# tauzn-clock/mpsfm

Measured on AMD Instinct MI355X. Metric: BA residual-evals/sec (LM iterations/sec alongside), 200 imgs / 150k pts prior-BA, higher is better.
Workload: dtype f64; 1 GPU; C3: 200 cameras, 150000 landmarks per rank, 749145 reprojection + 674306 log-depth blocks per rank, SoftL1/Cauchy, Ceres-default LM; parallelism=single GPU, residual_blocks_total=1423451

## Files before the change

### include/mpsfm_hip_debug.h

```cpp
#ifndef MPSFM_HIP_DEBUG_H
#define MPSFM_HIP_DEBUG_H

#include "mpsfm_hip.h"

#ifdef __cplusplus
extern "C" {
#endif

typedef struct mpsfm_plan_handle mpsfm_plan_handle;

void mpsfm_debug_set(int f);
int mpsfm_debug_set_chol_trace(long long* dev_buf);
int mpsfm_debug_panel_factor(const double* dx, int waves, double* out, int* ok);

mpsfm_plan_handle* mpsfm_debug_plan_create(const uint8_t* adj, int32_t n, int32_t depth, int32_t pinv_max_tiles, int32_t inv_rows);
void mpsfm_debug_plan_destroy(mpsfm_plan_handle* h);
int64_t mpsfm_debug_plan_get(const mpsfm_plan_handle* h, int32_t what, int32_t* out, int64_t cap);

int64_t mpsfm_debug_host_cache(int64_t bytes, int32_t count);
int64_t mpsfm_debug_run_parts(int32_t nparts, int32_t reps);
int mpsfm_debug_graph_union(const uint8_t* adj, int32_t world, int32_t n, uint8_t* out);

int mpsfm_debug_pt_handoff(mpsfm_ba_handle* h);
int mpsfm_debug_dense_solve_given(mpsfm_ba_handle* h, const double* S, const double* rhs, int32_t n, int32_t* failed);
int mpsfm_debug_read_trace(mpsfm_ba_handle* h, long long* out, int64_t count);
int64_t mpsfm_debug_table(mpsfm_ba_handle* h, int32_t which, void* out, int64_t cap);
int64_t mpsfm_debug_host_build(const mpsfm_ba_problem* P, int32_t which, void* out, int64_t cap);
int mpsfm_debug_local_clocks(mpsfm_ba_handle* h, int64_t out[12]);
int mpsfm_debug_local_skew(int32_t chunk, int32_t phase_mask, int64_t ticks);
int mpsfm_debug_resources(int32_t device, int64_t out[5]);

#ifdef __cplusplus
}
#endif
#endif
```

### mpsfm_amd/abi.py

```python

from __future__ import annotations

import ctypes as C
import os

MAX_TRACE = 64
INT_MAX_IRLS = 16

TERMINATION_NAMES = {
    0: "function_tolerance",
    1: "gradient_tolerance",
    2: "parameter_tolerance",
    3: "max_iterations",
    4: "min_radius",
    5: "invalid_steps",
    6: "no_variables",
}

ALLREDUCE_FN = C.CFUNCTYPE(C.c_int, C.c_void_p, C.POINTER(C.c_double), C.c_int64, C.c_int, C.c_void_p)


class CProblem(C.Structure):
    _c_name_ = "mpsfm_ba_problem"
    _fields_ = [
# ... 315 lines not shown

SIGNATURES = {
    "mpsfm_abi_version": (C.c_int, []),
    "mpsfm_last_error": (C.c_char_p, []),
    "mpsfm_device_count": (C.c_int, []),
    "mpsfm_ba_default_options": (None, [P]),
    "mpsfm_comm_unique_id": (C.c_int, [P]),
    "mpsfm_ba_solve": (C.c_int, [P, P, P, P]),
    "mpsfm_ba_create": (C.c_int, [P, P, P, _pp]),
    "mpsfm_ba_set_state": (C.c_int, [P, P]),
    "mpsfm_ba_reset_state": (C.c_int, [P]),
    "mpsfm_ba_solve_resident": (C.c_int, [P, P]),
    "mpsfm_ba_get_state": (C.c_int, [P, P]),
    "mpsfm_ba_destroy": (None, [P]),
    "mpsfm_ba_eval_cost": (C.c_int, [P, _f64p, _f64p]),
    "mpsfm_ba_sweep_once": (C.c_int, [P, F64, _f32p]),
    "mpsfm_ba_sweep_parts": (C.c_int, [P, P, P]),
    "mpsfm_ba_get_reduced_system": (C.c_int, [P, P, P, I32]),
    "mpsfm_ba_reduced_dim": (C.c_int, [P]),
    "mpsfm_ba_get_dense_solution": (C.c_int, [P, P, I32]),
    "mpsfm_ba_dense_solve_once": (C.c_int, [P, _f32p]),
    "mpsfm_ba_dense_plan": (C.c_int, [P, P]),
    "mpsfm_point_covs": (C.c_int, [P, P, I32, P]),
    "mpsfm_triangulate_tracks": (C.c_int, [P, I32, P]),
    "mpsfm_filter_tracks": (C.c_int, [P, P, I32, P, P, P]),
    "mpsfm_tri_default_options": (None, [P]),
    "mpsfm_triangulator_create": (C.c_int, [P, I32, _pp]),
    "mpsfm_triangulator_destroy": (None, [P]),
    "mpsfm_triangulator_set_state": (C.c_int, [P, P]),
    "mpsfm_triangulator_triangulate_image": (C.c_int, [P, P, I32, _i64p]),
    "mpsfm_triangulator_complete_image": (C.c_int, [P, P, I32, _i64p]),
    "mpsfm_triangulator_complete_tracks": (C.c_int, [P, P, P, I64, _i64p]),
    "mpsfm_triangulator_merge_tracks": (C.c_int, [P, P, P, I64, _i64p]),
    "mpsfm_triangulator_retriangulate": (C.c_int, [P, P, P, I32, _i64p]),
    "mpsfm_triangulator_num_ops": (I64, [P]),
    "mpsfm_triangulator_num_points": (I64, [P]),
    "mpsfm_triangulator_get_ops": (C.c_int, [P, P, P, P, P]),
    "mpsfm_triangulator_num_op_elements": (I64, [P]),
    "mpsfm_triangulator_get_op_elements": (C.c_int, [P, P]),
    "mpsfm_triangulator_stats": (C.c_int, [P, _i64p, _i64p, _i64p]),
    "mpsfm_tri_estimate_batch": (C.c_int, [P, I32, P, P, P]),
    "mpsfm_depth_blocks": (C.c_int, [P, I32, P, P, P, P, P, P]),
    "mpsfm_integrate_depth": (C.c_int, [P, I32, P, P]),
    "mpsfm_integrate_depth_batch": (C.c_int, [I32, P, I32, P, P]),
    "mpsfm_integration_variances": (C.c_int, [P, I32, I32, I32, P, P, F64, I32, P, P, P]),
    "mpsfm_depth_consistency": (C.c_int, [I32, P, I32, P, P, F64, F64, I32, P, P, P]),
    "mpsfm_abs_pose_estimate": (C.c_int, [I64, P, P, P, P, I32, P, P]),
    "mpsfm_rel_pose_estimate": (C.c_int, [I64, P, P, P, P, P, I32, P, P]),
    "mpsfm_two_view_default_options": (None, [P]),
    "mpsfm_two_view_geometry": (C.c_int, [I64, P, P, P, P, P, P, P, I32, P, P]),
    "mpsfm_two_view_geometry_batch": (C.c_int, [I64, P, P, P, P, P, P, P, P, I32, I32, P, P, P]),
    "mpsfm_registration_pairs": (C.c_int, [I32, P, I64, P, P, P, P, I32, P, I32, I32, P, P, P]),
    "mpsfm_init_pair_candidates": (C.c_int, [P, I32, P]),
    "mpsfm_radius_nms": (C.c_int, [I64, P, P, P, F64, I32, P, P, P]),
    "mpsfm_thin_dense_matches": (C.c_int, [I64, P, P, I64, P, P, P, F64, I32, I32, P, P, P]),
    "mpsfm_assign_keypoints": (C.c_int, [I64, P, I64, P, F64, I32, P, P]),
    "mpsfm_match_default_options": (None, [P]),
    "mpsfm_match_descriptors": (C.c_int, [I64, I64, I32, P, P, P, I32, P, P, P]),
    "mpsfm_match_descriptors_batch": (C.c_int, [I32, P, I32, P, I64, P, P, P, P, I32, I32, I32, P, P, P, P]),
    "mpsfm_match_map_descriptors": (C.c_int, [P, P, I32, I32, P, P, I32, I32, I32, I64, P, I64, P, P, I32, P, P, P]),
    "mpsfm_recip_default_options": (None, [P]),
    "mpsfm_recip_seed_count": (I64, [I32, I32, I32]),
    "mpsfm_reciprocal_nns": (C.c_int, [P, I32, I32, P, I32, I32, I32, P, I32, I64, P, P, P, P]),
    "mpsfm_dense_correspondences": (C.c_int, [P, P, P, P, P, P, P, P, I32, I32, I32, I32, I32, P, I32, I64, P, P, P, P, P]),
    "mpsfm_warp_default_options": (None, [P]),
    "mpsfm_simple_nms": (C.c_int, [I32, I32, P, I32, I32, P, I32, P, P]),
    "mpsfm_kpids_to_matches0": (C.c_int, [I64, P, P, P, I64, I64, I32, P, I32, P, P, P, P]),
    "mpsfm_warp_matches": (C.c_int, [I32, I32, P, P, I32, I32, I32, I32, I32, P, I64, P, I64, P, I32, P, P, P, P, P, P, P, P]),
    "mpsfm_depth_priors": (C.c_int, [I32, P, P, I32, P, P]),
    "mpsfm_normal_priors": (C.c_int, [I32, P, P, I32, P, P]),
}

DEBUG_SIGNATURES = {
    "mpsfm_debug_set": (None, [C.c_int]),
    "mpsfm_debug_set_chol_trace": (C.c_int, [P]),
    "mpsfm_debug_panel_factor": (C.c_int, [P, C.c_int, P, C.POINTER(C.c_int)]),
    "mpsfm_debug_plan_create": (P, [P, I32, I32, I32, I32]),
    "mpsfm_debug_plan_destroy": (None, [P]),
    "mpsfm_debug_plan_get": (I64, [P, I32, P, I64]),
    "mpsfm_debug_host_cache": (I64, [I64, I32]),
    "mpsfm_debug_run_parts": (I64, [I32, I32]),
    "mpsfm_debug_graph_union": (C.c_int, [P, I32, I32, P]),
    "mpsfm_debug_pt_handoff": (C.c_int, [P]),
    "mpsfm_debug_dense_solve_given": (C.c_int, [P, P, P, I32, C.POINTER(I32)]),
    "mpsfm_debug_read_trace": (C.c_int, [P, P, I64]),
    "mpsfm_debug_table": (I64, [P, I32, P, I64]),
    "mpsfm_debug_host_build": (I64, [P, I32, P, I64]),
    "mpsfm_debug_local_clocks": (C.c_int, [P, P]),
    "mpsfm_debug_local_skew": (C.c_int, [I32, I32, I64]),
    "mpsfm_debug_resources": (C.c_int, [I32, P]),
}


LIB_PATH = os.path.join(os.path.dirname(os.path.abspath(__file__)), "libmpsfm_hip.so")

_lib = None


class MpsfmHipError(RuntimeError):
    def __init__(self, code: int, msg: str):
        super().__init__(f"libmpsfm_hip error {code}: {msg}")
        self.code = code


def lib():
    global _lib
    if _lib is None:
        if not os.path.exists(LIB_PATH):
            raise MpsfmHipError(-2, f"{LIB_PATH} is missing: run `python -m mpsfm_amd.build` (hipcc, gfx950)")
        try:
            import torch
        except ImportError:
            pass
        L = C.CDLL(LIB_PATH)
        for table in (SIGNATURES, DEBUG_SIGNATURES):
            for name, (restype, argtypes) in table.items():
                fn = getattr(L, name)
                fn.restype, fn.argtypes = restype, argtypes
        _lib = L
    return _lib
```

### mpsfm_amd/capi.py

```python

from __future__ import annotations

import ctypes as C

import numpy as np

from .abi import (
    ALLREDUCE_FN, LIB_PATH, SIGNATURES, CAbsPoseOptions, CAbsPoseResult, CDcImage, CDcSummary, CDepthGather, CDepthPriorConf,
    CDepthPriorOutput, CDepthPriorProblem, CInitCandidates, CInitPair, CIntProblem, CIntSummary, CMatchBatchReport, CMatchInfo, CMatchOptions, CNmsInfo,
    CNormalPriorConf, CNormalPriorOutput, CNormalPriorProblem, COptions, CPriorSummary, CProblem, CRansacOptions, CRecipInfo,
    CRecipOptions, CRegImage, CRelPoseOptions, CRelPoseResult, CState, CSummary, CTracks, CTriCandidates, CTwoViewBatchReport, CTwoViewLeg, CTwoViewOptions,
    CTwoViewResult, CWarpInfo, CWarpOptions, MpsfmHipError, lib,
)
from .problem import BAProblem, Tracks

EXPORTS = list(SIGNATURES)
_MATCH_DESC_ARGS = SIGNATURES["mpsfm_match_descriptors"][1]
_MATCH_MAP_ARGS = SIGNATURES["mpsfm_match_map_descriptors"][1]
_SIMPLE_NMS_ARGS = SIGNATURES["mpsfm_simple_nms"][1]
_KPIDS_ARGS = SIGNATURES["mpsfm_kpids_to_matches0"][1]
_WARP_ARGS = SIGNATURES["mpsfm_warp_matches"][1]


def _check(rc: int):
# ... 37 lines not shown
_open_handles: "weakref.WeakSet" = None


def _track(handle):
    global _open_handles
    import atexit
    import weakref

    if _open_handles is None:
        _open_handles = weakref.WeakSet()

        def _close_all():
            for h in list(_open_handles):
                try:
                    h.close()
                except Exception:
                    pass

        atexit.register(_close_all)
    _open_handles.add(handle)


class BAHandle:

    def __init__(self, prob: BAProblem, options: COptions | None = None):
        self._h = C.c_void_p(None)
        self.prob = prob
        self.options = options if options is not None else default_options()
        cp, cs = prob.c_problem(), prob.c_state()
        _check(lib().mpsfm_ba_create(C.byref(cp), C.byref(cs), C.byref(self.options), C.byref(self._h)))
        _track(self)

    def close(self):
        if self._h:
            lib().mpsfm_ba_destroy(self._h)
            self._h = C.c_void_p(None)

    def __del__(self):
        try:
            self.close()
        except Exception:
            pass

    def __enter__(self):
        return self

    def __exit__(self, *a):
        self.close()

    def set_state(self, prob: BAProblem | None = None):
        cs = (prob or self.prob).c_state()
        _check(lib().mpsfm_ba_set_state(self._h, C.byref(cs)))

    def reset_state(self):
        _check(lib().mpsfm_ba_reset_state(self._h))

    def solve(self) -> dict:
        sm = CSummary()
        _check(lib().mpsfm_ba_solve_resident(self._h, C.byref(sm)))
        return sm.to_dict()

    def get_state(self, prob: BAProblem | None = None):
        cs = (prob or self.prob).c_state()
        _check(lib().mpsfm_ba_get_state(self._h, C.byref(cs)))

    def eval_cost(self) -> tuple[float, float]:
        a, b = C.c_double(0), C.c_double(0)
        _check(lib().mpsfm_ba_eval_cost(self._h, C.byref(a), C.byref(b)))
        return a.value, b.value

    @property
    def reduced_dim(self) -> int:
        return int(lib().mpsfm_ba_reduced_dim(self._h))

    def dense_plan(self) -> dict:
        v = (C.c_int64 * 10)()
        _check(lib().mpsfm_ba_dense_plan(self._h, v))
        keys = ["slots", "tile_columns", "levels", "nd_depth", "inverse_accumulators", "work_items", "tile_products", "inverse_roles",
                "s_blocks", "backsub_launches"]
        return dict(zip(keys, (int(x) for x in v)))

    def pt_handoff(self) -> bool:
        return bool(lib().mpsfm_debug_pt_handoff(self._h))

    def sweep_once(self, radius: float = 1e4) -> float:
        ms = C.c_float(0)
        _check(lib().mpsfm_ba_sweep_once(self._h, radius, C.byref(ms)))
        return ms.value

    def sweep_parts(self) -> dict:
        ms, info = (C.c_float * 3)(), (C.c_int64 * 4)()
        _check(lib().mpsfm_ba_sweep_parts(self._h, ms, info))
        return dict(dense_ms=ms[0], reduce_ms=ms[1], general_ms=ms[2], dense_chunks=int(info[0]), general_chunks=int(info[1]),
                    long_tracks=int(info[2]), reduce_parts=int(info[3]))

    def dense_solve_once(self) -> float:
        ms = C.c_float(0)
        _check(lib().mpsfm_ba_dense_solve_once(self._h, C.byref(ms)))
        return ms.value

    def dense_solve_given(self, S: np.ndarray, rhs: np.ndarray) -> bool:
        n = self.reduced_dim
        S, rhs = np.ascontiguousarray(S, np.float64), np.ascontiguousarray(rhs, np.float64)
        assert S.shape == (n, n) and rhs.shape == (n,)
        failed = C.c_int32(0)
        _check(lib().mpsfm_debug_dense_solve_given(self._h, S.ctypes.data, rhs.ctypes.data, n, C.byref(failed)))
        return bool(failed.value)

    def reduced_system(self):
        n = self.reduced_dim
        S, rhs = np.zeros((n, n)), np.zeros(n)
        _check(lib().mpsfm_ba_get_reduced_system(self._h, S.ctypes.data, rhs.ctypes.data, n))
        return S, rhs

    def dense_solution(self):
        n = self.reduced_dim
        y = np.zeros(n)
        _check(lib().mpsfm_ba_get_dense_solution(self._h, y.ctypes.data, n))
        return y


def ba_solve(prob: BAProblem, options: COptions | None = None) -> dict:
    o = options if options is not None else default_options()
    cp, cs, sm = prob.c_problem(), prob.c_state(), CSummary()
    _check(lib().mpsfm_ba_solve(C.byref(cp), C.byref(cs), C.byref(o), C.byref(sm)))
    return sm.to_dict()


def point_covs(prob: BAProblem, device: int = 0) -> np.ndarray:
    covs = np.zeros((prob.n_pts, 3, 3))
    cp, cs = prob.c_problem(), prob.c_state()
    _check(lib().mpsfm_point_covs(C.byref(cp), C.byref(cs), device, covs.ctypes.data))
    return covs


def debug_panel_factor(dx: np.ndarray, waves: int = 4):
    dx = np.ascontiguousarray(dx, np.float64)
    assert dx.shape == (64, 32), dx.shape
    out, ok = np.zeros((64, 32)), C.c_int(0)
    _check(lib().mpsfm_debug_panel_factor(dx.ctypes.data, int(waves), out.ctypes.data, C.byref(ok)))
    return out, bool(ok.value)


def debug_resources(device: int = 0) -> tuple:
    out = np.zeros(5, np.int64)
    _check(lib().mpsfm_debug_resources(int(device), out.ctypes.data))
    return tuple(int(v) for v in out)


def triangulate_tracks(tr: Tracks, device: int = 0) -> np.ndarray:
    xyz = np.zeros((tr.n_tracks, 3))
    ct = tr.c_tracks()
    _check(lib().mpsfm_triangulate_tracks(C.byref(ct), device, xyz.ctypes.data))
    return xyz


def filter_tracks(tr: Tracks, xyz: np.ndarray, device: int = 0):
    xyz = np.ascontiguousarray(xyz, np.float64)
    ang, err, front = np.zeros(tr.n_tracks), np.zeros(tr.n_el), np.zeros(tr.n_el, np.uint8)
    ct = tr.c_tracks()
    _check(lib().mpsfm_filter_tracks(C.byref(ct), xyz.ctypes.data, device, ang.ctypes.data, err.ctypes.data, front.ctypes.data))
    return ang, err, front.astype(bool)


def depth_blocks(depth_maps, valid_maps, sx, sy, cam_quat, cam_t, obs_img, obs_xy, obs_var, obs_pt, pts, scale_filter_factor=1.5,
                 multiplier=2.0, device=0):
# ... 938 lines not shown
```

### mpsfm_amd/csrc/ba_build.hip

```cpp
#include <algorithm>
#include <chrono>
#include <cstdio>
#include <cstring>
#include <mutex>
#include <string>
#include <vector>

#include "ba_handle.h"

namespace mpsfm {

void free_handle(mpsfm_ba_handle* h) {
  if (!h) return;
  (void)hipSetDevice(h->device);
  comm_destroy(h->comm);
  delete h;
}

int check_problem(const mpsfm_ba_problem* P) {
  if (!P) return fail(MPSFM_EINVAL, "problem is NULL");
  if (P->n_cams < 0 || P->n_pts < 0 || P->n_intr < 0 || P->n_obs < 0 || P->n_dobs < 0) return fail(MPSFM_EINVAL, "negative size");
  if (P->n_cams > 0 && (!P->cam_intr_idx || !P->pose_const || !P->cam_intr)) return fail(MPSFM_EINVAL, "camera arrays are NULL");
  if (P->n_pts > 0 && !P->pt_const) return fail(MPSFM_EINVAL, "pt_const is NULL");
  if (P->n_obs > 0 && (!P->obs_cam || !P->obs_pt || !P->obs_xy)) return fail(MPSFM_EINVAL, "observation arrays are NULL");
  if (P->n_dobs > 0 && (!P->dobs_cam || !P->dobs_pt || !P->dobs_depth || !P->dobs_magnitude || !P->dobs_param))
    return fail(MPSFM_EINVAL, "depth observation arrays are NULL");
  if (P->gauge_axis_cam < -1 || P->gauge_axis_cam >= P->n_cams) return fail(MPSFM_EINVAL, "gauge_axis_cam out of range");
  for (int i = 0; i < P->n_cams; ++i)
    if (P->cam_intr_idx[i] < 0 || P->cam_intr_idx[i] >= P->n_intr) return fail(MPSFM_EINVAL, "cam_intr_idx out of range");
  auto out_of_range = [](const int32_t* v, int64_t n, int32_t bound) {
    uint32_t bad = 0;
    const uint32_t b = (uint32_t)bound;
    for (int64_t i = 0; i < n; ++i) bad |= (uint32_t)((uint32_t)v[i] >= b);
    return bad != 0;
  };
  if (out_of_range(P->obs_cam, P->n_obs, P->n_cams) || out_of_range(P->obs_pt, P->n_obs, P->n_pts))
    return fail(MPSFM_EINVAL, "observation index out of range");
  if (out_of_range(P->dobs_cam, P->n_dobs, P->n_cams) || out_of_range(P->dobs_pt, P->n_dobs, P->n_pts))
    return fail(MPSFM_EINVAL, "depth observation index out of range");
  for (int t : {P->reproj_loss_type, P->depth_loss_type})
    if (t < MPSFM_LOSS_TRIVIAL || t > MPSFM_LOSS_CAUCHY) return fail(MPSFM_EINVAL, "unknown loss type");
  return 0;
}

void level_plan_flags(const CholPlan& PL, LevelPlanDev& D) { D.valid = PL.nt >= 1 && PL.nlevels >= 1; D.use_pinv = PL.use_pinv; }

static int upload_pattern(mpsfm_ba_handle* h, bool use_graph) {
  const CholPlan& PL = h->plan;
  DeviceBlocks& own = h->own;
  h->sky.ns = h->ncv;
  if (int rc = use_graph ? own.upload(&h->sky.index, h->spat.sky_index) : own.upload(&h->sky.first, h->spat.sky_first, &h->sky.start, h->spat.sky_start))
    return rc;
  std::vector<uint8_t> live((size_t)(PL.nt + 1) * (size_t)(PL.nt + 2) / 2, 0);
  for (int32_t id : PL.asm_tiles) live[(size_t)id] = 1;
  LevelPlanDev& D = h->lp;
  if (int rc = own.upload(&D.d_items, PL.items, &D.d_heads, PL.heads, &D.d_srcs, PL.srcs, &D.d_rows, PL.rows, &D.d_struct_start, PL.struct_start,
                          &D.d_struct_rows, PL.struct_rows, &D.d_back_cols, PL.back_cols, &D.d_asm_tiles, PL.asm_tiles,
                          &D.d_col_slot, PL.slot_of_col, &D.d_tile_live, live))
    return rc;
  if (PL.slot_of_col.empty()) D.d_col_slot = nullptr;
  level_plan_flags(PL, D);
  D.n_asm = (int32_t)PL.asm_tiles.size(); D.nlevels = PL.nlevels;
  D.h_launch_start = PL.launch_start.data(); D.h_back_start = PL.back_start.data();
  return 0;
}


static void graph_from_stage1(const std::vector<uint64_t>& gbits, int words, const std::vector<int32_t>& prov, int nprov, const CameraLayout& cams,
                              CamGraph& graph) {
  graph.init(cams.ncv_real);
  std::vector<int32_t> nat_of_prov((size_t)std::max(nprov, 1), -1);
  for (size_t i = 0; i < cams.slot.size(); ++i) if (prov[i] >= 0) nat_of_prov[(size_t)prov[i]] = cams.slot[i];
  for (int a = 0; a < nprov; ++a) {
    const int na = nat_of_prov[(size_t)a];
    for (int w = 0; w < words; ++w) {
      uint64_t m = gbits[(size_t)a * words + w];
      while (m) {
        const int b = w * 64 + __builtin_ctzll(m);
        m &= m - 1;
        const int nb = nat_of_prov[(size_t)b];
        if (na >= 0 && nb >= 0) graph.set(na, nb);
      }
    }
  }
}

static int pair_tables_of_device_build(hipStream_t stream, const mpsfm_ba_problem* P, const RecTablesDev& rt, HostTables& T, const Lap& lap) {
  std::vector<ChunkHdr>& chunks = T.chunks;
  size_t g0 = 0;
  while (g0 < chunks.size() && chunks[g0].dense) ++g0;
  T.blk_ent_start.assign(g0, 0);
  if (g0 == chunks.size()) return 0;
  const int64_t r0 = chunks[g0].rec0, k0 = chunks[g0].pt0, nrg = T.nrec - r0, nkg = T.np_chunked - k0;
  std::vector<uint32_t> rm((size_t)std::max<int64_t>(nrg, 1));
  std::vector<uint16_t> kvs((size_t)std::max<int64_t>(nkg, 1));
  std::vector<int32_t> prs((size_t)std::max<int64_t>(nkg, 1));
  MPSFM_TRY(hipMemcpyAsync(rm.data(), rt.rec_meta + r0, 4 * (size_t)nrg, hipMemcpyDeviceToHost, stream));
  MPSFM_TRY(hipMemcpyAsync(kvs.data(), rt.pt_kv + k0, 2 * (size_t)nkg, hipMemcpyDeviceToHost, stream));
  MPSFM_TRY(hipMemcpyAsync(prs.data(), rt.pt_rec_start + k0, 4 * (size_t)nkg, hipMemcpyDeviceToHost, stream));
  MPSFM_TRY(hipStreamSynchronize(stream));
  PairScratch ps;
  for (size_t c = g0; c < chunks.size(); ++c) {
    if (chunks[c].dense) return fail(MPSFM_EUNSUPPORTED, "internal: dense chunks must precede the general ones");
    append_pair_tables(chunks[c], rm.data() - r0, kvs.data() - k0, prs.data() - k0, T.order.data(), P->pt_const, T.blk_desc, T.ents, T.blk_ent_start, ps);
  }
  if (T.ents.size() > (size_t)INT32_MAX) return fail(MPSFM_EUNSUPPORTED, "too many Schur pairs for 32-bit entry offsets");
  lap("pair tables of the general chunks (host)");
  return 0;
}

static void print_chunk_stats(const std::vector<ChunkHdr>& chunks) {
  double sr = 0, sp = 0, sc = 0, sb = 0, se = 0, sd = 0; int mb = 0, mc = 0;
  for (const ChunkHdr& H : chunks) { sr += H.nrec; sp += H.npt; sc += H.ncam; sb += H.nblk; se += H.nent; sd += H.dense; mb = std::max(mb, H.nblk); mc = std::max(mc, H.ncam); }
  const double n = (double)chunks.size();
  std::fprintf(stderr, "[mpsfm_ba] build: %zu chunks; per chunk: %.1f records, %.1f landmarks, %.1f cameras (max %d), %.1f work items (max %d), %.1f pairs; %.0f %% of the chunks take the dense product\n",
               chunks.size(), sr / n, sp / n, sc / n, mc, sb / n, mb, se / n, 100.0 * sd / n);
  int hist[kDenseCams + 2] = {0};
  for (const ChunkHdr& H : chunks) ++hist[std::min<int>(H.ncam, kDenseCams + 1)];
  std::fprintf(stderr, "[mpsfm_ba] build: chunks by number of variable cameras:");
  for (int c = 0; c <= kDenseCams + 1; ++c) std::fprintf(stderr, " %s%d: %d", c > kDenseCams ? ">" : "", c > kDenseCams ? kDenseCams : c, hist[c]);
  std::fprintf(stderr, "\n");
}

static int upload_tables(mpsfm_ba_handle* h, const mpsfm_ba_problem* P, const CameraLayout& cams, DevBuildOut& DB, SlabTables& R, DevBuilder* devb,
                         bool slab_tables_on_device) {
  HostTables& T = DB.t;
  const int nc = P->n_cams;
  int rc = 0;
  DeviceBlocks& own = h->own;
  std::vector<double> intr(P->cam_intr, P->cam_intr + (size_t)P->n_intr * 4);
  std::vector<int32_t> intr_idx(P->cam_intr_idx, P->cam_intr_idx + nc);
  if ((rc = own.upload(&h->d_intr, intr, &h->d_intr_idx, intr_idx, &h->d_cmask, cams.cmask, &h->d_cam_slot, h->cam_slot_h,
                       &h->d_cam_of_slot, cam_of_slot_table(cams), &h->d_chunks, T.chunks, &h->d_chunk_cams, T.chunk_cams)))
    return rc;
  if (h->np > 0 && h->np == (int64_t)h->np_user) {
    if ((rc = own.upload(&h->d_perm, h->perm))) return rc;
    if ((rc = own.alloc(&h->d_user_pts, (size_t)h->np * 3))) return rc;
  }
  if (h->built_on_device) {
    h->rt = DB.rt;
    own.adopt(std::move(DB.own));
    own.drop(DB.d_chunks); own.drop(DB.d_chunk_cams);
  } else {
    RecTablesDev& rt = h->rt;
    if ((rc = own.upload(&rt.rec_cam, T.rec_cam, &rt.rec_pt, T.rec_pt, &rt.rec_meta, T.rec_meta, &rt.rec_xy, T.rec_xy, &rt.rec_d, T.rec_d, &rt.rec_m, T.rec_m,
                         &rt.rec_a, T.rec_a, &rt.pt_rec_start, T.pt_rec_start, &rt.pt_kv, T.pt_kv, &rt.fx_cam, T.fx_cam, &rt.fx_pt, T.fx_pt,
                         &rt.fx_meta, T.fx_meta, &rt.fx_xy, T.fx_xy, &rt.fx_d, T.fx_d, &rt.fx_m, T.fx_m, &rt.fx_a, T.fx_a)))
      return rc;
  }
  if ((rc = own.upload(&h->d_lhdr, T.lhdr))) return rc;
  if ((rc = own.alloc(&h->d_wl, (size_t)std::max<int64_t>(T.wl_rows, 1) * 18))) return rc;
  h->n_blk_desc = (int64_t)T.blk_desc.size(); h->n_blk_ent_start = (int64_t)T.blk_ent_start.size(); h->n_ents = (int64_t)T.ents.size();
  if ((rc = own.upload(&h->d_blk_desc, T.blk_desc, &h->d_blk_ent_start, T.blk_ent_start, &h->d_ents, T.ents))) return rc;
  int32_t* d_diag_block = nullptr;
  if (!slab_tables_on_device) {
    if ((rc = own.upload(&h->d_red_dests, R.dests, &h->d_red_srcs, R.srcs))) return rc;
  } else if ((rc = own.upload(&d_diag_block, R.diag_block))) return rc;
  if ((rc = own.alloc(&h->d_slab, (size_t)std::max<int64_t>(R.slab_units, 1) * 18))) return rc;

  if ((rc = staged_drain())) return rc;
  if (slab_tables_on_device) {
    if ((rc = devb->slab_tables(h->d_chunks, h->n_dense, h->d_chunk_cams, h->sky, h->spat.nblk, h->ncv, d_diag_block, own, &h->d_red_dests, &h->n_red_dests,
                                &h->d_red_srcs, &h->n_red_srcs)))
      return rc;
    MPSFM_TRY(hipStreamSynchronize(h->stream));
    own.drop(d_diag_block);
  }
  return 0;
}

static int alloc_work_buffers(mpsfm_ba_handle* h, const BuildOptions& opt) {
  int rc = 0;
  DeviceBlocks& own = h->own;
  const size_t ncs = (size_t)std::max(h->nc, 1), nps = (size_t)std::max<int64_t>(h->np, 1);
  for (double** p : {&h->d_q, &h->d_q2, &h->d_q0}) if ((rc = own.alloc(p, ncs * 4))) return rc;
  for (double** p : {&h->d_t, &h->d_t2, &h->d_t0}) if ((rc = own.alloc(p, ncs * 3))) return rc;
  for (double** p : {&h->d_pts, &h->d_pts2, &h->d_pts0, &h->d_ps, &h->d_diagV}) if ((rc = own.alloc(p, nps * 3))) return rc;
  if (h->nlong == 0 && h->n_dense > 0 && h->n_dense == h->nchunks) if ((rc = own.alloc(&h->d_pt_fac, nps * 9))) return rc;
  if ((rc = own.alloc(&h->d_cs, ncs * 6))) return rc;
  if ((rc = own.alloc(&h->d_camtab, ncs * kCamRec))) return rc;
  if ((rc = own.alloc(&h->d_camtab2, ncs * kCamRec))) return rc;
  h->sblk_count = h->spat.nblk * 36;
  h->red_count = h->sblk_count + 3 * (int64_t)h->n_user + SC_COUNT;
  if ((rc = own.alloc(&h->d_red, (size_t)h->red_count))) return rc;
  h->d_Sblk = h->d_red; h->d_gc = h->d_red + h->sblk_count; h->d_wv = h->d_gc + h->n_user; h->d_diagU = h->d_wv + h->n_user;
  h->d_redsc = h->d_diagU + h->n_user;
  if ((rc = own.alloc(&h->d_part, (size_t)std::max(h->nchunks + h->nlong, 1) * 4 * 2))) return rc;
  if ((rc = own.alloc(&h->d_part2, (size_t)std::max(h->nchunks + h->nlong, 1) * 8))) return rc;
  if ((rc = own.alloc(&h->d_scal, (size_t)U_COUNT))) return rc;
  if ((rc = own.alloc(&h->d_costpart, (size_t)1024 * 4))) return rc;
  static_assert(sizeof(double) * U_COUNT * 2 <= kPinnedBytes, "pinned scalar block too small");
  MPSFM_TRY(own.pinned((void**)&h->h_scal));
  static_assert(sizeof(LmCtl) * 2 <= kPinnedBytes, "pinned block too small for two control-block copies");
  MPSFM_TRY(own.pinned((void**)&h->h_ctl));
  if ((rc = own.alloc(&h->d_ctl, 1))) return rc;
  for (auto& e : h->ev2) MPSFM_TRY(own.event(&e, true));
  const size_t ntiles = (size_t)(h->nt + 1) * (h->nt + 2) / 2;
  if ((rc = own.alloc(&h->d_A, ntiles * 1024))) return rc;
  if ((rc = own.alloc(&h->d_dwork, dense_work_doubles(h->nt)))) return rc;
  if ((rc = own.alloc(&h->d_yc, (size_t)std::max(h->n_user, 1)))) return rc;
  if ((rc = own.alloc(&h->d_fail, 1))) return rc;
  MPSFM_TRY(hipMemsetAsync(h->d_fail, 0, sizeof(int), h->stream));
  for (auto& e : h->ev) MPSFM_TRY(own.event(&e, true));
  opt.apply_dense(h->nt, h->plan, h->ov);
  if (h->nt > 64 || h->ov.nb > 0) {
    MPSFM_TRY(own.stream(&h->ov.s2));
    for (auto& e : h->ov.evF) MPSFM_TRY(own.event(&e, false));
    for (auto& e : h->ov.evB) MPSFM_TRY(own.event(&e, false));
  }
  h->local_ok = false;
  if (opt.local_lm && !sharded(h) && h->nlong == 0 && h->nchunks > 0 && h->n_dense == h->nchunks && h->ncv >= 1 && h->ncv <= kLocalCams &&
      h->n_user == 6 * h->ncv && h->nchunks <= local_lm_max_chunks(h->device)) {
    h->local_log_cap = std::max(h->opt.max_num_iterations, 0) + 2;
    if ((rc = own.alloc(&h->d_local_acc, (size_t)2 * kLocalAccDoubles))) return rc;
    if ((rc = own.alloc(&h->d_local_sync, (size_t)16))) return rc;
    if ((rc = own.alloc(&h->d_local_log, (size_t)h->local_log_cap))) return rc;
    h->local_ok = true;
  }
  MPSFM_TRY(hipMemsetAsync(h->d_ps, 0, nps * 3 * sizeof(double), h->stream));
  MPSFM_TRY(hipMemsetAsync(h->d_yc, 0, (size_t)std::max(h->n_user, 1) * sizeof(double), h->stream));
  MPSFM_TRY(hipStreamSynchronize(h->stream));
  return 0;
}

int build_tables(const mpsfm_ba_problem* P, BuildOptions& opt, const SumExchange& exchange, bool sharded, int verbose, const Lap& lap, DeviceStages* devs,
                 TableBuild& out) {
  const int nc = P->n_cams;
  CameraLayout& cams = out.cams;
  HostTables& T = out.tables.t;

  bool dev = false;
  std::vector<uint64_t> dev_gbits;
  std::vector<int32_t> prov((size_t)std::max(nc, 1), -1);
  int nprov = 0;
  for (int i = 0; i < nc; ++i) if (!P->pose_const[i]) prov[(size_t)i] = nprov++;
  const int dev_words = (nprov + 63) / 64;
  std::vector<double> cnt(nc + 1, 0.0);
  if (devs && !sharded && nprov <= kIndexMaxSlots && nc <= 8192 && P->n_obs + P->n_dobs > 0 && opt.dev_build && opt.chol_graph) {
    devs->builder.reset(new DevBuilder());
    int64_t max_blocks = 0;
    if (int rc = devs->builder->stage1(P, devs->stream, prov, nprov, cnt, dev_gbits, dev_words, &max_blocks)) return rc;
    dev = max_blocks <= kObsMax;
    lap("device stage 1 (upload, group, graph)");
  } else {
    count_camera_blocks(P, cnt);
    if (exchange) if (int rc = exchange(cnt.data(), nc)) return rc;
  }
  assign_camera_slots(P, cnt, opt, cams);
  opt.set_chunk_caps(sharded, cams.ncv, P->n_obs);

  LandmarkGroups groups;
  if (!dev) if (int rc = group_blocks_by_landmark(P, true, groups)) return rc;
  lap("group blocks by landmark (threads)");

  CamGraph graph;
  if (cams.use_graph) {
    if (dev) graph_from_stage1(dev_gbits, dev_words, prov, nprov, cams, graph);
    else camera_graph_from_groups(P, groups, cams, graph);
    if (exchange) if (int rc = union_graph_over_ranks(graph, exchange)) return rc;
    lap("camera graph");
    plan_camera_order(graph, opt, out.plan, cams);
    lap("camera order + factorisation plan");
  } else keep_caller_order(cams);

  if (dev) {
    const int rc2 = devs->builder->stage2(cams.slot, opt.sweep_dense, opt.rec_cap, opt.pts_by_cams, out.tables);
    if (rc2 < 0) return rc2;
    if (rc2 == MPSFM_DEVBUILD_FALLBACK) {
      dev = false;
      if (int rc = group_blocks_by_landmark(P, false, groups)) return rc;
      lap("device build not applicable: host phases");
    } else {
      if (T.nrec > (int64_t)INT32_MAX) return fail(MPSFM_EUNSUPPORTED, "more than 2^31 records on one device");
      lap("device stage 2 (order, chunks, records)");
      if (int rc = pair_tables_of_device_build(devs->stream, P, out.tables.rt, T, lap)) return rc;
    }
  }
  if (!dev) if (int rc = build_record_tables(P, cams, opt, groups, T, lap)) return rc;
  out.built_on_device = dev;
  {
    double tot[3] = {(double)(P->n_obs + P->n_dobs), (double)T.nblk_reduced, T.nvarpts};
    if (exchange) if (int rc = exchange(tot, 3)) return rc;
    out.nblocks_global = tot[0]; out.nblocks_reduced_global = tot[1]; out.nvarpts_global = tot[2];
  }
  lap("chunks + pair tables");
  if (verbose >= 2 && !T.chunks.empty()) print_chunk_stats(T.chunks);

  if (cams.use_graph) s_pattern_index(cams, out.plan, graph, out.spat);
  else if (int rc = s_pattern_skyline(cams, T, opt, exchange, verbose >= 2, out.spat, out.plan)) return rc;
  if (verbose >= 2) {
    const CholPlan& PL = out.plan;
    std::fprintf(stderr, "[mpsfm_ba] build: camera order: %s (depth %d), %d slots for %d cameras, %d tile columns in %d levels, %lld tile products, %lld inverse roles, %d blocks of S\n",
                 PL.nd_depth < 0 ? "caller's" : "nested dissection", PL.nd_depth, PL.nslots, PL.ncv, PL.nt, PL.nlevels, (long long)PL.products, (long long)PL.roles, (int)out.spat.nblk);
  }

  SlabTables& slabs = out.slabs;
  if (int rc = assign_slabs(T.chunks, slabs)) return rc;
  out.slab_tables_on_device = dev && slabs.n_dense > 0 && (opt.slab_tables_host == 0 || (opt.slab_tables_host < 0 && slabs.n_dense >= 512));
  if (int rc = slab_reduction_tables(T, cams, out.plan, out.spat, !out.slab_tables_on_device, slabs)) return rc;
  lap("slab reduction tables");
  return 0;
}

static int build(mpsfm_ba_handle* h, const mpsfm_ba_problem* P) {
  const Lap lap = stopwatch(h->opt.verbose >= 2, "[mpsfm_ba] build: %-28s %8.2f ms\n");
  h->nc = P->n_cams; h->np_user = P->n_pts;
  h->loss.reproj_type = P->reproj_loss_type; h->loss.reproj_a = P->reproj_loss_scale;
  h->loss.reproj_mag = P->reproj_loss_magnitude; h->loss.depth_type = P->depth_loss_type;
  BuildOptions opt = BuildOptions::from_environment();
  const SumExchange exchange = sharded(h) ? SumExchange([h](double* buf, int64_t count) { return allreduce_host(h, buf, count); }) : SumExchange();
  DeviceStages devs{h->stream, nullptr};
  TableBuild B;
  if (int rc = build_tables(P, opt, exchange, sharded(h), h->opt.verbose, lap, &devs, B)) return rc;

  h->plan = std::move(B.plan); h->spat = std::move(B.spat);
  const CameraLayout& cams = B.cams;
  HostTables& T = B.tables.t;
  h->n_user = 6 * cams.ncv_real;
  h->cam_slot_h = cams.slot; h->nat_slot = cams.nat_slot;
  h->ncv = cams.ncv; h->n = cams.n; h->nt = cams.nt;
  h->built_on_device = B.built_on_device;
  h->np = T.np; h->np_chunked = T.np_chunked; h->nfixed = T.nfixed; h->nrec = T.nrec;
  h->nchunks = (int)T.chunks.size(); h->nlong = (int)T.lhdr.size();
  h->nblocks_total = P->n_obs + P->n_dobs; h->nblocks_reduced = T.nblk_reduced;
  h->nblocks_global = B.nblocks_global; h->nblocks_reduced_global = B.nblocks_reduced_global; h->nvarpts_global = B.nvarpts_global;
  h->n_dense = B.slabs.n_dense; h->n_red_dests = (int)B.slabs.dests.size();
  h->n_red_srcs = (int64_t)B.slabs.srcs.size(); h->n_chunk_cams = (int64_t)T.chunk_cams.size();
  h->perm.swap(T.order);

  if (int rc = upload_pattern(h, cams.use_graph)) return rc;
  if (int rc = upload_tables(h, P, cams, B.tables, B.slabs, devs.builder.get(), B.slab_tables_on_device)) return rc;
  lap("upload tables");
  if (int rc = alloc_work_buffers(h, opt)) return rc;
  lap("allocate work buffers");
  return 0;
}

int upload_state(mpsfm_ba_handle* h, const mpsfm_ba_state* st, bool as_initial) {
  if (!st || (h->nc > 0 && (!st->cam_quat_xyzw || !st->cam_t)) || (h->np > 0 && !st->pts)) return fail(MPSFM_EINVAL, "state is NULL");
  const Lap lap = stopwatch(h->opt.verbose >= 2, "[mpsfm_ba] state: %-28s %8.2f ms\n");
  MPSFM_TRY(hipStreamSynchronize(h->stream));
  lap("stream idle");
  if (h->nc > 0) {
    if (int rc = staged_h2d(h->d_q, st->cam_quat_xyzw, sizeof(double) * 4 * h->nc)) return rc;
    if (int rc = staged_h2d(h->d_t, st->cam_t, sizeof(double) * 3 * h->nc)) return rc;
  }
  lap("pose copies");
  if (h->d_perm) {
    if (int rc = staged_h2d(h->d_user_pts, st->pts, sizeof(double) * 3 * h->np)) return rc;
    launch_permute_pts(h->np, h->d_perm, h->d_user_pts, h->d_pts, false, h->stream);
    lap("landmark copy + permute (device)");
  } else {
    std::vector<double> sorted((size_t)h->np * 3);
    parallel_ranges(h->np, 16384, [&](int64_t k0, int64_t k1) {
      for (int64_t k = k0; k < k1; ++k) {
        const double* s = st->pts + 3 * (size_t)h->perm[(size_t)k];
        sorted[3 * (size_t)k] = s[0]; sorted[3 * (size_t)k + 1] = s[1]; sorted[3 * (size_t)k + 2] = s[2];
      }
    });
    lap("permute landmarks");
    if (h->np > 0) if (int rc = staged_h2d(h->d_pts, sorted.data(), sizeof(double) * 3 * h->np)) return rc;
  }
  lap("landmark copy");
  if (as_initial) {
    MPSFM_TRY(hipMemcpyAsync(h->d_q0, h->d_q, sizeof(double) * 4 * h->nc, hipMemcpyDeviceToDevice, h->stream));
    MPSFM_TRY(hipMemcpyAsync(h->d_t0, h->d_t, sizeof(double) * 3 * h->nc, hipMemcpyDeviceToDevice, h->stream));
    if (h->np > 0) MPSFM_TRY(hipMemcpyAsync(h->d_pts0, h->d_pts, sizeof(double) * 3 * h->np, hipMemcpyDeviceToDevice, h->stream));
    MPSFM_TRY(hipStreamSynchronize(h->stream));
    lap("keep initial state");
  }
  h->scales_ready = false;
  return 0;
}

int create_impl(const mpsfm_ba_problem* P, const mpsfm_ba_state* st, const mpsfm_ba_options* o, mpsfm_ba_handle** out) {
  if (!out) return fail(MPSFM_EINVAL, "out is NULL");
  *out = nullptr;
  const auto t_begin = std::chrono::steady_clock::now();
  auto since = [&](const char* what) {
    if (o && o->verbose >= 2)
      std::fprintf(stderr, "[mpsfm_ba] create: %-27s %8.2f ms (cumulative)\n", what,
                   1e3 * std::chrono::duration<double>(std::chrono::steady_clock::now() - t_begin).count());
  };
  if (int rc = check_problem(P)) return rc;
  if (!o) return fail(MPSFM_EINVAL, "options is NULL");
  since("check_problem");
  int ndev = 0;
  if (hipGetDeviceCount(&ndev) != hipSuccess || ndev <= 0) return fail(MPSFM_ENODEVICE, "no HIP device visible: libmpsfm_hip has no CPU fallback");
  if (o->device < 0 || o->device >= ndev) return fail(MPSFM_EINVAL, "device ordinal out of range");
  if (o->device >= kMaxDevices) return fail(MPSFM_EUNSUPPORTED, "device ordinals beyond 15 are not supported (per-device pools)");
  {
    static std::mutex mu;
    static std::vector<std::string> arch;
    std::lock_guard<std::mutex> lk(mu);
    if ((int)arch.size() < ndev) arch.resize((size_t)ndev);
    if (arch[(size_t)o->device].empty()) {
      hipDeviceProp_t prop;
      MPSFM_TRY(hipGetDeviceProperties(&prop, o->device));
      arch[(size_t)o->device] = prop.gcnArchName;
    }
    if (std::strncmp(arch[(size_t)o->device].c_str(), "gfx950", 6) != 0)
      return fail(MPSFM_ENODEVICE, std::string("device is ") + arch[(size_t)o->device] + ", this library is built for gfx950 only");
  }
  since("device check");
  MPSFM_TRY(hipSetDevice(o->device));
  mpsfm_ba_handle* h = new mpsfm_ba_handle();
  h->device = o->device; h->opt = *o;
  if (o->stream) { h->stream = (hipStream_t)o->stream; h->own.idle_first(h->stream); }
  else if (h->own.stream(&h->stream) != hipSuccess) { delete h; return fail(MPSFM_EHIP, "hipStreamCreate failed"); }
  if (o->use_rccl && o->world_size >= 1) {
    if (int rc = comm_init_rank(h)) { free_handle(h); return rc; }
    since("ncclCommInitRank");
  }
  int rc = build(h, P);
  since("build");
  if (rc == 0 && st) rc = upload_state(h, st, true);
  since("upload_state");
// ... 7 lines not shown
```

### mpsfm_amd/csrc/ba_debug.hip

```cpp
#include <algorithm>
#include <atomic>
#include <cstring>
#include <vector>

#include "../../include/mpsfm_hip_debug.h"
#include "ba_handle.h"

using namespace mpsfm;

static void dense_plan_numbers(int ncv, int nt, const CholPlan& P, const DenseOverlap& ov, const LevelPlanDev& lp, double* work, int64_t sblk, int64_t v[10]) {
  const bool level = dense_level(&ov, &lp);
  const bool pinv = level && dense_pinv(work, nt, &ov, &lp) != nullptr;
  const int64_t w[10] = {ncv, nt, level ? P.nlevels : nt, P.nd_depth, pinv ? 1 : 0, (int64_t)P.items.size(), P.products, P.roles, sblk,
                         pinv ? 1 : (level ? P.nlevels : (nt + 3) / 4 + 1)};
  for (int i = 0; i < 10; ++i) v[i] = w[i];
}

extern "C" int64_t mpsfm_debug_host_cache(int64_t bytes, int32_t count) {
  std::vector<mpsfm::HostBuf<uint8_t>> first((size_t)count), second((size_t)count);
  std::vector<const void*> seen;
  for (auto& b : first) { b.alloc((size_t)bytes); b[0] = 1; b[(size_t)bytes - 1] = 2; seen.push_back(b.data()); }
  first.clear();
  int64_t reused = 0;
  for (auto& b : second) {
    b.alloc((size_t)bytes);
    b[0] = 3;
    reused += std::find(seen.begin(), seen.end(), (const void*)b.data()) != seen.end() ? 1 : 0;
  }
  return reused;
}

extern "C" int64_t mpsfm_debug_run_parts(int32_t nparts, int32_t reps) {
  int64_t bad = 0;
  for (int r = 0; r < reps; ++r) {
    std::vector<std::atomic<int>> hits((size_t)std::max(nparts, 1));
    for (auto& x : hits) x.store(0);
    mpsfm::run_parts(nparts, [&](int t, int np) {
      if (np != std::max(nparts, 1) || t < 0 || t >= np) return;
      volatile double acc = 0.0;
      for (int k = 0; k < 2000; ++k) acc = acc + (double)k * 1e-9;
      hits[(size_t)t].fetch_add(1);
    });
    for (auto& x : hits) bad += x.load() == 1 ? 0 : 1;
  }
  return bad;
}

extern "C" int mpsfm_debug_graph_union(const uint8_t* adj, int32_t world, int32_t n, uint8_t* out) {
  std::vector<double> sum;
  for (int r = 0; r < world; ++r) {
    mpsfm::CamGraph g;
    g.init(n);
    for (int a = 0; a < n; ++a)
      for (int b = 0; b < n; ++b)
        if (adj[((size_t)r * n + a) * n + b]) g.set(a, b);
    std::vector<double> packed;
    mpsfm::pack_graph(g, world, packed);
    if (sum.empty()) sum.assign(packed.size(), 0.0);
    for (size_t i = 0; i < packed.size(); ++i) sum[i] += packed[i];
  }
  mpsfm::CamGraph u;
  u.init(n);
  mpsfm::unpack_graph(sum, world, u);
  for (int a = 0; a < n; ++a)
    for (int b = 0; b < n; ++b) out[(size_t)a * n + b] = u.get(a, b) ? 1 : 0;
  return mpsfm::graph_digits(world);
}

extern "C" {

int mpsfm_ba_dense_plan(mpsfm_ba_handle* h, int64_t info[10]) {
  if (!h || !info) return fail(MPSFM_EINVAL, "handle or info is NULL");
  dense_plan_numbers(h->ncv, h->nt, h->plan, h->ov, h->lp, h->d_dwork, h->spat.nblk, info);
  return 0;
}

int mpsfm_debug_pt_handoff(mpsfm_ba_handle* h) { return h && h->d_pt_fac != nullptr ? 1 : 0; }

int mpsfm_ba_sweep_once(mpsfm_ba_handle* h, double radius, float* elapsed_ms) {
  if (!h) return fail(MPSFM_EINVAL, "handle is NULL");
  MPSFM_TRY(hipSetDevice(h->device));
  if (!h->scales_ready) if (int rc = prepare_scales(h)) return rc;
  MPSFM_TRY(hipMemsetAsync(h->d_red, 0, sizeof(double) * (size_t)h->red_count, h->stream));
  SweepArgs a = sweep_args(h, radius);
  MPSFM_TRY(hipEventRecord(h->ev[0], h->stream));
  launch_track_sweep_dense(a, h->n_dense, h->stream);
  MPSFM_TRY(hipEventRecord(h->ev[1], h->stream));
  launch_reduce_slabs(h->d_red_dests, h->n_red_dests, h->d_red_srcs, h->d_slab, h->d_Sblk, h->d_gc, h->d_wv, h->d_diagU, nullptr, h->stream);
  MPSFM_TRY(hipEventRecord(h->ev[2], h->stream));
  a.chunk0 = h->n_dense;
  launch_track_sweep(a, h->nchunks - h->n_dense, false, h->stream);
  MPSFM_TRY(hipEventRecord(h->ev[3], h->stream));
  if (h->nchunks + h->nlong > 0) launch_reduce_cols(h->d_part, h->nchunks + h->nlong, 4, 3, 1u << 2, h->d_redsc, h->stream);
  MPSFM_TRY(hipStreamSynchronize(h->stream));
  MPSFM_TRY(hipGetLastError());
  h->last_radius = radius;
  float ms = 0.f;
  MPSFM_TRY(hipEventElapsedTime(&ms, h->ev[0], h->ev[3]));
  if (elapsed_ms) *elapsed_ms = ms;
  return 0;
}

int mpsfm_debug_read_trace(mpsfm_ba_handle* h, long long* out, int64_t count) {
  if (!h || !out || count < 0 || count > 3 * std::max<int64_t>(h->np, 1)) return fail(MPSFM_EINVAL, "bad trace request");
  MPSFM_TRY(hipSetDevice(h->device));
  MPSFM_TRY(hipMemcpyAsync(out, h->d_diagV, sizeof(long long) * (size_t)count, hipMemcpyDeviceToHost, h->stream));
  MPSFM_TRY(hipStreamSynchronize(h->stream));
  return 0;
}

int64_t mpsfm_debug_table(mpsfm_ba_handle* h, int32_t which, void* out, int64_t cap) {
  if (!h) return fail(MPSFM_EINVAL, "handle is NULL");
  const void* src = nullptr;
  int64_t bytes = 0;
  bool host = false;
  const int64_t nr = h->nrec, np1 = h->np + 1, nf = h->nfixed;
  switch (which) {
    case 0: src = h->d_chunks; bytes = (int64_t)sizeof(ChunkHdr) * h->nchunks; break;
    case 1: src = h->d_chunk_cams; bytes = 4 * h->n_chunk_cams; break;
    case 2: src = h->rt.rec_cam; bytes = 4 * nr; break;
    case 3: src = h->rt.rec_pt; bytes = 4 * nr; break;
    case 4: src = h->rt.rec_meta; bytes = 4 * nr; break;
    case 5: src = h->rt.rec_xy; bytes = 16 * nr; break;
    case 6: src = h->rt.rec_d; bytes = 8 * nr; break;
    case 7: src = h->rt.rec_m; bytes = 8 * nr; break;
    case 8: src = h->rt.rec_a; bytes = 8 * nr; break;
    case 9: src = h->rt.pt_rec_start; bytes = 4 * np1; break;
    case 10: src = h->rt.pt_kv; bytes = 2 * np1; break;
    case 11: src = h->rt.fx_cam; bytes = 4 * nf; break;
    case 12: src = h->rt.fx_pt; bytes = 4 * nf; break;
    case 13: src = h->rt.fx_meta; bytes = 4 * nf; break;
    case 14: src = h->rt.fx_xy; bytes = 16 * nf; break;
    case 15: src = h->rt.fx_d; bytes = 8 * nf; break;
    case 16: src = h->rt.fx_m; bytes = 8 * nf; break;
    case 17: src = h->rt.fx_a; bytes = 8 * nf; break;
    case 18: src = h->perm.data(); bytes = 4 * (int64_t)h->perm.size(); host = true; break;
    case 19: src = h->d_red_dests; bytes = (int64_t)sizeof(RedDest) * h->n_red_dests; break;
    case 20: src = h->d_red_srcs; bytes = 4 * h->n_red_srcs; break;
    case 21: src = h->cam_slot_h.data(); bytes = 4 * (int64_t)h->cam_slot_h.size(); host = true; break;
    case 23: src = h->d_blk_desc; bytes = 4 * h->n_blk_desc; break;
    case 24: src = h->d_blk_ent_start; bytes = 4 * h->n_blk_ent_start; break;
    case 25: src = h->d_ents; bytes = 4 * h->n_ents; break;
    case 26: src = h->d_part; bytes = 32 * (int64_t)h->nchunks; break;
    case 22: { static uint8_t flag; flag = h->built_on_device ? 1 : 0; src = &flag; bytes = 1; host = true; break; }
    case 27: src = h->d_lhdr; bytes = (int64_t)sizeof(LongHdr) * h->nlong; break;
    case 28: src = h->spat.sky_index.data(); bytes = 4 * (int64_t)h->spat.sky_index.size(); host = true; break;
    case 29: src = h->spat.sky_first.data(); bytes = 4 * (int64_t)h->spat.sky_first.size(); host = true; break;
    case 30: src = h->spat.sky_start.data(); bytes = 8 * (int64_t)h->spat.sky_start.size(); host = true; break;
    case 31: src = h->d_cmask; bytes = 48 * (int64_t)h->nc; break;
    case 32: src = h->d_cam_of_slot; bytes = 4 * (int64_t)std::max(h->ncv, 1); break;
    case 33: { static thread_local int64_t info[10]; if (int rc = mpsfm_ba_dense_plan(h, info)) return rc; src = info; bytes = 80; host = true; break; }
    case 34: src = h->last_launches; bytes = (int64_t)sizeof(h->last_launches); host = true; break;
    default: return fail(MPSFM_EINVAL, "unknown table");
  }
  if (!out || cap < bytes) return bytes;
  if (bytes == 0) return 0;
  if (host) { std::memcpy(out, src, (size_t)bytes); return bytes; }
  if (hipSetDevice(h->device) != hipSuccess) return fail(MPSFM_EHIP, "hipSetDevice failed");
  if (hipMemcpyAsync(out, src, (size_t)bytes, hipMemcpyDeviceToHost, h->stream) != hipSuccess) return fail(MPSFM_EHIP, "copy failed");
  if (hipStreamSynchronize(h->stream) != hipSuccess) return fail(MPSFM_EHIP, "sync failed");
// ... 184 lines not shown
```

### mpsfm_amd/csrc/ba_handle.h

```cpp
#pragma once
#include <cstdint>
#include <memory>
#include <vector>

#include "ba_launch.h"
#include "build_host.h"
#include "common.h"
#include "dev_resources.h"
#include "devbuild.h"

struct mpsfm_ba_handle {
  int device = 0;
  mpsfm::DeviceBlocks own;
  hipStream_t stream = nullptr;
  void* comm = nullptr;
  mpsfm::DenseOverlap ov;
  mpsfm::SPattern spat;
  mpsfm::BlockSky sky{nullptr, nullptr, nullptr, 0};
  mpsfm::CholPlan plan;
  mpsfm::LevelPlanDev lp;
  std::vector<int32_t> nat_slot;
  int n_user = 0;
  mpsfm_ba_options opt{};
  mpsfm::LossParams loss{};
  int nc = 0, np_user = 0;
  int64_t np = 0, np_chunked = 0;
  int64_t nrec = 0, nfixed = 0, nblocks_total = 0, nblocks_reduced = 0;
  double nblocks_global = 0, nblocks_reduced_global = 0, nvarpts_global = 0;
  int ncv = 0, n = 0, nt = 0, nchunks = 0, nlong = 0;
  int n_dense = 0;
  double* d_slab = nullptr;
  mpsfm::RedDest* d_red_dests = nullptr;
  int32_t* d_red_srcs = nullptr;
  int n_red_dests = 0;
  int64_t n_red_srcs = 0, n_chunk_cams = 0, n_blk_desc = 0, n_blk_ent_start = 0, n_ents = 0;
  bool built_on_device = false;
  mpsfm::LongHdr* d_lhdr = nullptr;
  double* d_wl = nullptr;
  int64_t red_count = 0, sblk_count = 0;
  std::vector<int32_t> perm;
  int32_t* d_cam_of_slot = nullptr;
  int32_t* d_perm = nullptr;
  double* d_user_pts = nullptr;
  std::vector<int32_t> cam_slot_h;
  double *d_q = nullptr, *d_t = nullptr, *d_q2 = nullptr, *d_t2 = nullptr, *d_q0 = nullptr, *d_t0 = nullptr;
  double *d_pts = nullptr, *d_pts2 = nullptr, *d_pts0 = nullptr;
  double *d_intr = nullptr, *d_cmask = nullptr, *d_cs = nullptr, *d_camtab = nullptr, *d_camtab2 = nullptr;
  int32_t *d_intr_idx = nullptr, *d_cam_slot = nullptr;
  double *d_ps = nullptr, *d_diagV = nullptr;
  double* d_pt_fac = nullptr;
  mpsfm::ChunkHdr* d_chunks = nullptr;
  int32_t *d_chunk_cams = nullptr, *d_blk_ent_start = nullptr;
  uint32_t *d_blk_desc = nullptr, *d_ents = nullptr;
  mpsfm::RecTablesDev rt;
  double* d_red = nullptr;
  double *d_Sblk = nullptr, *d_gc = nullptr, *d_wv = nullptr, *d_diagU = nullptr, *d_redsc = nullptr;
  double *d_part = nullptr, *d_part2 = nullptr, *d_scal = nullptr, *d_costpart = nullptr;
  double* h_scal = nullptr;
  mpsfm::LmCtl* d_ctl = nullptr;
  mpsfm::LmCtl* h_ctl = nullptr;
  hipEvent_t ev2[4] = {nullptr, nullptr, nullptr, nullptr};
  double *d_A = nullptr, *d_yc = nullptr, *d_dwork = nullptr;
  int* d_fail = nullptr;
  hipEvent_t ev[4] = {nullptr, nullptr, nullptr, nullptr};
  double last_radius = 1e4;
  bool scales_ready = false;
  int64_t last_launches[mpsfm::kLfCount] = {};
  double split_front_s = 0.0;
  bool local_ok = false;
  double* d_local_acc = nullptr;
  int64_t* d_local_sync = nullptr;
  mpsfm::LmHead* d_local_log = nullptr;
  int local_log_cap = 0;
};

namespace mpsfm {

inline bool sharded(const mpsfm_ba_handle* h) { return h->opt.allreduce != nullptr || h->comm != nullptr; }

struct TableBuild {
  CameraLayout cams;
  CholPlan plan;
  SPattern spat;
  DevBuildOut tables;
  SlabTables slabs;
  double nblocks_global = 0, nblocks_reduced_global = 0, nvarpts_global = 0;
  bool built_on_device = false;
  bool slab_tables_on_device = false;
};
struct DeviceStages {
  hipStream_t stream = nullptr;
  std::unique_ptr<DevBuilder> builder;
};

int check_problem(const mpsfm_ba_problem* P);
int build_tables(const mpsfm_ba_problem* P, BuildOptions& opt, const SumExchange& exchange, bool sharded, int verbose, const Lap& lap, DeviceStages* dev,
                 TableBuild& out);
void level_plan_flags(const CholPlan& PL, LevelPlanDev& D);

int create_impl(const mpsfm_ba_problem* P, const mpsfm_ba_state* st, const mpsfm_ba_options* o, mpsfm_ba_handle** out);
int upload_state(mpsfm_ba_handle* h, const mpsfm_ba_state* st, bool as_initial);
void free_handle(mpsfm_ba_handle* h);

int comm_init_rank(mpsfm_ba_handle* h);
void comm_destroy(void* comm);
int allreduce_host(mpsfm_ba_handle* h, double* buf, int64_t count);
int allreduce_dev(mpsfm_ba_handle* h, double* buf, int64_t count);

SweepArgs sweep_args(mpsfm_ba_handle* h, double radius, const LmCtl* ctl = nullptr);
int prepare_scales(mpsfm_ba_handle* h);
int run_track_sweep(mpsfm_ba_handle* h, double radius, const LmCtl* ctl = nullptr, bool in_loop = false, bool adopt = false, bool handoff = false);
void run_assemble(mpsfm_ba_handle* h, double radius, const LmCtl* ctl = nullptr);
int run_dense(mpsfm_ba_handle* h, double radius, const LmCtl* ctl = nullptr);
bool chol_entry_list();

struct LocalSkew { int32_t chunk = 0, mask = 0; int64_t ticks = 0; };
extern LocalSkew g_local_skew;

}
```

### mpsfm_amd/csrc/ba_launch.h

```cpp
#pragma once
#include "common.h"
#include "local_lm.h"

namespace mpsfm {
enum LaunchFamily {
  kLfTrackSweep,
  kLfReduceSlabs,
  kLfAssemble,
  kLfCholLevel,
  kLfDenseRest,
  kLfUpdateSweep,
  kLfDecide,
  kLfScales,
  kLfOther,
  kLfCount
};
extern thread_local int64_t g_launches[kLfCount];
inline void count_launch(LaunchFamily f, int n = 1) { g_launches[f] += n; }

void launch_track_sweep(const SweepArgs&, int nchunks, bool diag_only, hipStream_t);
void launch_update_sweep(const SweepArgs&, int nchunks, hipStream_t, const CamUpdArgs* cu = nullptr);
void launch_track_sweep_dense(const SweepArgs&, int nchunks, hipStream_t);
void launch_reduce_slabs(const RedDest* dests, int ndest, const int32_t* srcs, const double* slab, double* Sblk, double* gc, double* wv, double* diagU,
                         const LmCtl* ctl, hipStream_t);
void launch_cost_records(const CostArgs&, int nblocks, hipStream_t);
void launch_reduce_cols(const double* part, int64_t rows, int stride, int ncols, uint32_t max_mask, double* out, hipStream_t,
                        double* out2 = nullptr, int gmax_slot = -1);
void launch_build_camtab(int nc, const double* q, const double* t, const double* intr, const int32_t* intr_idx,
                         const double* cs, double* camtab, hipStream_t);
void launch_cam_scales(int nc, const int32_t* cam_slot, const double* cmask, const double* diagU, int jacobi, double* cs, hipStream_t);
void launch_pt_scales(int64_t np, const uint16_t* pt_kv, const double* diagV, int jacobi, double* ps, hipStream_t);
void launch_cam_update(int nc, const int32_t* cam_slot, const double* q, const double* t, const double* cs, const double* yc,
                       const double* gc, double* q2, double* t2, double* scal, hipStream_t, const double* intr = nullptr,
                       const int32_t* intr_idx = nullptr, double* camtab2 = nullptr, int* chol_fail = nullptr, const LmCtl* ctl = nullptr);
void launch_lm_decide(LmCtl* ctl, double* scal, const LmOpts& o, LmCtl* host_copy, hipStream_t, const double* redsc = nullptr);
void launch_zero(double* p, int64_t n, const LmCtl* ctl, hipStream_t);
void launch_lm_reduce_decide(const double* part, const double* part2, int64_t rows, LmCtl* ctl, double* scal, const LmOpts& o, LmCtl* host_copy, hipStream_t);
void launch_lm_prologue(const LmCtl* ctl, double* red, int64_t nred, int nc, int64_t np, double* q, double* t, double* camtab, double* pts, const double* q2,
                        const double* t2, const double* camtab2, const double* pts2, hipStream_t);
void launch_lm_accept(const LmCtl* ctl, int nc, int64_t np, double* q, double* t, double* camtab, double* pts, const double* q2, const double* t2,
                      const double* camtab2, const double* pts2, hipStream_t);
void launch_pts_sqnorm(int64_t np, const uint16_t* pt_kv, const double* pts, double* part, int nblocks, hipStream_t);
void launch_gmax_to_slot(double* redsc, int rank, hipStream_t);
void launch_lm_pack(const double* scal, double* sums, hipStream_t);
void launch_lm_init(LmCtl* ctl, const double* scal, const double* sums, hipStream_t);
void launch_permute_pts(int64_t np, const int32_t* perm, const double* src, double* dst, bool scatter, hipStream_t);
void launch_gmax_from_slots(const double* redsc, double* scal, hipStream_t);

extern int g_dbg_flags;
void launch_assemble(const AssembleArgs&, hipStream_t);
void launch_dense_solve(double* A, double* work, int nt, int n, double* y, int* fail, hipStream_t, DenseOverlap* ov, const LevelPlanDev* lp,
                        const LmCtl* ctl = nullptr);
bool dense_level(const DenseOverlap* ov, const LevelPlanDev* lp);
int dense_plain_max_tiles();
int dense_inv_rows();
size_t dense_work_doubles(int nt);
double* dense_pinv(double* work, int nt, const DenseOverlap* ov, const LevelPlanDev* lp);

int local_lm_max_chunks(int device);
int launch_local_lm(const LocalArgs& a, hipStream_t s);

}
```

### mpsfm_amd/csrc/ba_solver.hip

```cpp
#include <algorithm>
#include <chrono>
#include <cstdio>
#include <cstdlib>
#include <cstring>
#include <vector>

#include "ba_handle.h"

namespace mpsfm {

LocalSkew g_local_skew;

SweepArgs sweep_args(mpsfm_ba_handle* h, double radius, const LmCtl* ctl) {
  SweepArgs a{};
  a.ctl = ctl;
  a.chunks = h->d_chunks; a.chunk_cams = h->d_chunk_cams; a.rec_cam = h->rt.rec_cam; a.rec_meta = h->rt.rec_meta;
  a.rec_xy = h->rt.rec_xy; a.rec_d = h->rt.rec_d; a.rec_m = h->rt.rec_m; a.rec_a = h->rt.rec_a;
  a.pt_rec_start = h->rt.pt_rec_start; a.pt_kv = h->rt.pt_kv; a.blk_desc = h->d_blk_desc; a.blk_ent_start = h->d_blk_ent_start; a.ents = h->d_ents;
  a.camtab = h->d_camtab; a.pts = h->d_pts; a.ps = h->d_ps; a.loss = h->loss;
  a.radius = radius; a.min_diag = h->opt.min_lm_diagonal; a.max_diag = h->opt.max_lm_diagonal; a.ncv = h->ncv; a.dbg = (g_dbg_flags >> 8) & 0xff;
  a.lhdr = h->d_lhdr; a.nlong = h->nlong; a.nchunks = h->nchunks; a.cam_slot = h->d_cam_slot; a.wl = h->d_wl;
  a.sky = h->sky;
  a.Sblk = h->d_Sblk; a.gc = h->d_gc; a.wv = h->d_wv; a.diagU = h->d_diagU; a.part = h->d_part; a.diagV = h->d_diagV;
  a.yc = h->d_yc; a.camtab2 = h->d_camtab2; a.pts2 = h->d_pts2; a.part2 = h->d_part2;
  a.slab = h->d_slab; a.chunk0 = 0;
  return a;
}

static void launch_record_cost(mpsfm_ba_handle* h, bool fixed, double* out) {
  const RecTablesDev& r = h->rt;
  const int64_t nrec = fixed ? h->nfixed : h->nrec;
  const int nb = (int)std::min<int64_t>(1024, (nrec + kThreads - 1) / kThreads);
  const CostArgs c = fixed ? CostArgs{nrec, r.fx_cam, r.fx_pt, r.fx_meta, r.fx_xy, r.fx_d, r.fx_m, r.fx_a, h->d_camtab, h->d_pts, h->loss, h->d_costpart}
                           : CostArgs{nrec, r.rec_cam, r.rec_pt, r.rec_meta, r.rec_xy, r.rec_d, r.rec_m, r.rec_a, h->d_camtab, h->d_pts, h->loss, h->d_costpart};
  launch_cost_records(c, nb, h->stream);
  launch_reduce_cols(h->d_costpart, nb, 4, 3, 0u, out, h->stream);
}
static void launch_fixed_cost(mpsfm_ba_handle* h, double* out) {
  if (h->nfixed > 0) launch_record_cost(h, true, out);
}
static int cost_of_records(mpsfm_ba_handle* h, bool fixed, double* out3) {
  out3[0] = out3[1] = out3[2] = 0.0;
  if ((fixed ? h->nfixed : h->nrec) <= 0) return 0;
  launch_record_cost(h, fixed, h->d_scal);
  MPSFM_TRY(hipMemcpyAsync(h->h_scal, h->d_scal, sizeof(double) * 3, hipMemcpyDeviceToHost, h->stream));
  MPSFM_TRY(hipStreamSynchronize(h->stream));
  out3[0] = h->h_scal[0]; out3[1] = h->h_scal[1]; out3[2] = h->h_scal[2];
  return 0;
}

int prepare_scales(mpsfm_ba_handle* h) {
  hipStream_t s = h->stream;
  launch_cam_scales(h->nc, h->d_cam_slot, h->d_cmask, h->d_diagU, 0, h->d_cs, s);
  launch_pt_scales(h->np, h->rt.pt_kv, h->d_diagV, 0, h->d_ps, s);
  launch_build_camtab(h->nc, h->d_q, h->d_t, h->d_intr, h->d_intr_idx, h->d_cs, h->d_camtab, s);
  if (h->opt.jacobi_scaling) {
    MPSFM_TRY(hipMemsetAsync(h->d_diagU, 0, sizeof(double) * (size_t)std::max(h->n_user, 1), s));
    MPSFM_TRY(hipMemsetAsync(h->d_diagV, 0, sizeof(double) * 3 * (size_t)std::max<int64_t>(h->np, 1), s));
    SweepArgs a = sweep_args(h, 1.0);
    launch_track_sweep(a, h->nchunks, true, s);
    if (int rc = allreduce_dev(h, h->d_diagU, h->n_user)) return rc;
    launch_cam_scales(h->nc, h->d_cam_slot, h->d_cmask, h->d_diagU, 1, h->d_cs, s);
    launch_pt_scales(h->np, h->rt.pt_kv, h->d_diagV, 1, h->d_ps, s);
    launch_build_camtab(h->nc, h->d_q, h->d_t, h->d_intr, h->d_intr_idx, h->d_cs, h->d_camtab, s);
  }
  MPSFM_TRY(hipGetLastError());
  h->scales_ready = true;
  return 0;
}

static void launch_sweeps(mpsfm_ba_handle* h, SweepArgs a, hipStream_t s) {
  launch_track_sweep_dense(a, h->n_dense, s);
  launch_reduce_slabs(h->d_red_dests, h->n_red_dests, h->d_red_srcs, h->d_slab, h->d_Sblk, h->d_gc, h->d_wv, h->d_diagU, a.ctl, s);
  a.chunk0 = h->n_dense;
  launch_track_sweep(a, h->nchunks - h->n_dense, false, s);
}

int run_track_sweep(mpsfm_ba_handle* h, double radius, const LmCtl* ctl, bool in_loop, bool adopt, bool handoff) {
  hipStream_t s = h->stream;
  if (!in_loop) launch_zero(h->d_red, h->red_count, ctl, s);
  SweepArgs a = sweep_args(h, radius, ctl);
  if (adopt) {
    a.adopt_on = 1; a.adopt_nc = h->nc;
    a.pts_rw = h->d_pts; a.q_rw = h->d_q; a.t_rw = h->d_t; a.camtab_rw = h->d_camtab; a.q2 = h->d_q2; a.t2 = h->d_t2;
    a.red = h->d_red; a.nred = h->red_count;
  }
  if (handoff) a.pt_fac = h->d_pt_fac;
  launch_sweeps(h, a, s);
  if (h->nchunks + h->nlong > 0 && !(in_loop && !sharded(h)))
    launch_reduce_cols(h->d_part, h->nchunks + h->nlong, 4, 3, 1u << 2, h->d_redsc, s, sharded(h) ? nullptr : h->d_scal + U_X_COST,
                       sharded(h) ? (h->opt.rank > 0 ? h->opt.rank : 0) % kMaxRankSlots : -1);
  else if (sharded(h)) launch_gmax_to_slot(h->d_redsc, h->opt.rank > 0 ? h->opt.rank : 0, s);
  h->last_radius = radius;
  return 0;
}

void run_assemble(mpsfm_ba_handle* h, double radius, const LmCtl* ctl) {
  const bool level = dense_level(&h->ov, &h->lp);
  double* pinv = dense_pinv(h->d_dwork, h->nt, &h->ov, &h->lp);
  const bool listed = level && !pinv;
  AssembleArgs as{h->sky, h->d_Sblk, h->d_gc, h->d_wv, h->d_diagU, h->ncv, h->n, h->nt, radius,
                  h->opt.min_lm_diagonal, h->opt.max_lm_diagonal, h->d_A, pinv, listed ? h->lp.d_asm_tiles : nullptr, listed ? h->lp.n_asm : 0,
                  h->lp.d_col_slot, h->n_user, (level && pinv) ? h->d_yc : nullptr, (level && pinv) ? h->lp.d_tile_live : nullptr, ctl};
  launch_assemble(as, h->stream);
}

int run_dense(mpsfm_ba_handle* h, double radius, const LmCtl* ctl) {
  if (h->n > 0) {
    run_assemble(h, radius, ctl);
    launch_dense_solve(h->d_A, h->d_dwork, h->nt, h->n, h->d_yc, h->d_fail, h->stream, &h->ov, &h->lp, ctl);
  }
  return 0;
}

static LmOpts lm_opts_of(const mpsfm_ba_options& o) {
  return LmOpts{o.function_tolerance, o.gradient_tolerance, o.parameter_tolerance, o.min_relative_decrease, o.max_trust_region_radius,
                o.min_trust_region_radius, o.max_num_iterations, o.max_num_consecutive_invalid_steps};
}
static LmCtl initial_ctl(const mpsfm_ba_options& o) {
  LmCtl c0;
  std::memset(&c0, 0, sizeof(c0));
  c0.radius = o.initial_trust_region_radius; c0.decrease_factor = 2.0;
  c0.term = kLmRunning; c0.check_gradient = 1;
  return c0;
}
static void print_iteration(int it, const LmHead& l, double fixed_cost) {
  if (l.last_mcc > 0.0 && l.last_cand != DBL_MAX)
    std::fprintf(stderr, "[mpsfm_ba] it %3d cost %.9e cand %.9e rel %.3e radius %.3e |step| %.3e\n", it, l.last_x_cost + fixed_cost, l.last_cand + fixed_cost,
                 l.last_rel, l.radius, l.last_step_norm);
  else
    std::fprintf(stderr, "[mpsfm_ba] it %3d invalid step (chol_fail=%d mcc=%.3e) radius %.3e\n", it, l.last_chol_fail, l.last_mcc, l.radius);
}
static int summary_from_ctl(mpsfm_ba_handle* h, const LmCtl& last, mpsfm_ba_summary* sum) {
  h->last_radius = last.radius;
  sum->num_jacobian_evals = last.n_jac_evals;
  sum->num_residual_evals = (int64_t)h->nblocks_reduced_global * ((int64_t)last.n_cost_evals + last.n_jac_evals);
  if (last.term == kLmNumericError)
    return fail(MPSFM_ENUMERIC, "the initial point cannot be evaluated (non-finite residual or depth <= 0 in a log-depth block)");
  sum->initial_cost = last.initial_cost;
  sum->fixed_cost = last.fixed_cost;
  sum->final_cost = last.cur_cost + last.fixed_cost;
  sum->num_iterations = last.iter;
  sum->num_successful_steps = last.n_success;
  sum->num_unsuccessful_steps = last.n_unsuccess;
  sum->termination = last.term;
  sum->final_radius = last.radius;
  sum->trace_len = last.trace_len;
  for (int i = 0; i < last.trace_len; ++i) { sum->trace_cost[i] = last.trace_cost[i]; sum->trace_radius[i] = last.trace_radius[i]; sum->trace_accepted[i] = last.trace_accepted[i]; }
  return 0;
}

constexpr int kLocalRefused = 1;
constexpr double kSplitMinFront = 40e-6;
bool chol_entry_list() { const char* e = std::getenv("MPSFM_CHOL_ENTRY"); return e && std::strcmp(e, "list") == 0; }
static bool pt_handoff_enabled() { const char* e = std::getenv("MPSFM_PT_HANDOFF"); return !(e && std::atoi(e) == 0); }

static int solve_local(mpsfm_ba_handle* h, mpsfm_ba_summary* sum) {
  hipStream_t s = h->stream;
  const mpsfm_ba_options& o = h->opt;
  launch_cam_scales(h->nc, h->d_cam_slot, h->d_cmask, h->d_diagU, 0, h->d_cs, s);
  launch_build_camtab(h->nc, h->d_q, h->d_t, h->d_intr, h->d_intr_idx, h->d_cs, h->d_camtab, s);
  double* fixed_parts = h->d_scal + 12;
  MPSFM_TRY(hipMemsetAsync(h->d_scal, 0, sizeof(double) * U_COUNT, s));
  launch_fixed_cost(h, fixed_parts);
  if (int rc = prepare_scales(h)) return rc;
  h->h_ctl[0] = initial_ctl(o);
  MPSFM_TRY(hipMemcpyAsync(h->d_ctl, &h->h_ctl[0], sizeof(LmCtl), hipMemcpyHostToDevice, s));
  MPSFM_TRY(hipMemsetAsync(h->d_local_acc, 0, sizeof(double) * 2 * kLocalAccDoubles, s));
  MPSFM_TRY(hipMemsetAsync(h->d_local_sync, 0, sizeof(int64_t) * 16, s));
  LocalArgs la{};
  la.A = sweep_args(h, 0.0, nullptr);
  if (pt_handoff_enabled()) la.A.pt_fac = h->d_pt_fac;
  la.ctl = h->d_ctl;
  la.o = lm_opts_of(o);
  la.log = o.verbose > 0 ? h->d_local_log : nullptr;
  la.acc[0] = h->d_local_acc; la.acc[1] = h->d_local_acc + kLocalAccDoubles;
  la.part[0] = h->d_part; la.part[1] = h->d_part + (size_t)h->nchunks * 4;
  la.bar = reinterpret_cast<int32_t*>(h->d_local_sync); la.clk = reinterpret_cast<long long*>(h->d_local_sync + 1);
  la.ncv = h->ncv; la.nc = h->nc; la.nchunks = h->nchunks;
  la.q = h->d_q; la.t = h->d_t; la.camtab = h->d_camtab; la.pts = h->d_pts; la.cs = h->d_cs; la.fixed_parts = fixed_parts;
  la.skew_chunk = g_local_skew.chunk; la.skew_mask = g_local_skew.ticks > 0 ? g_local_skew.mask : 0; la.skew_ticks = g_local_skew.ticks;
  if (launch_local_lm(la, s) != (int)hipSuccess) {
    (void)hipGetLastError();
    MPSFM_TRY(hipStreamSynchronize(s));
    return kLocalRefused;
  }
  static_assert(sizeof(int64_t) * 8 <= sizeof(double) * U_COUNT * 2, "the pinned scalar block holds the sync words");
  int64_t* hs = reinterpret_cast<int64_t*>(h->h_scal);
  MPSFM_TRY(hipMemcpyAsync(&h->h_ctl[0], h->d_ctl, sizeof(LmCtl), hipMemcpyDeviceToHost, s));
  MPSFM_TRY(hipMemcpyAsync(hs, h->d_local_sync, sizeof(int64_t) * 8, hipMemcpyDeviceToHost, s));
  MPSFM_TRY(hipStreamSynchronize(s));
  MPSFM_TRY(hipGetLastError());
  if (reinterpret_cast<const int32_t*>(hs)[1] != 0)
    return fail(MPSFM_EHIP, "single-launch solver: a grid barrier did not complete (workgroups not co-resident?); MPSFM_LOCAL_LM=0 selects the launch chain");
  const LmCtl& last = h->h_ctl[0];
  sum->fixed_cost = last.fixed_cost;
  sum->time_linearize_s = 1e-8 * (double)(hs[1] + hs[2]); sum->time_dense_s = 1e-8 * (double)hs[3]; sum->time_update_s = 1e-8 * (double)(hs[4] + hs[5] + hs[6]);
  if (o.verbose > 0) {
    const int nlog = std::min(last.iter + 1, h->local_log_cap);
    std::vector<LmHead> log((size_t)std::max(nlog, 0));
    if (nlog > 0) MPSFM_TRY(hipMemcpy(log.data(), h->d_local_log, sizeof(LmHead) * (size_t)nlog, hipMemcpyDeviceToHost));
    for (int i = 0; i < nlog; ++i)
      if (log[(size_t)i].iter == i + 1 || i == nlog - 1) print_iteration(i + 1, log[(size_t)i], last.fixed_cost);
  }
  return summary_from_ctl(h, last, sum);
}

static int solve_impl(mpsfm_ba_handle* h, mpsfm_ba_summary* sum) {
  using clk = std::chrono::steady_clock;
  MPSFM_TRY(hipSetDevice(h->device));
  hipStream_t s = h->stream;
  const mpsfm_ba_options& o = h->opt;
  std::memset(sum, 0, sizeof(*sum));
  MPSFM_TRY(hipStreamSynchronize(s));
  const auto t_begin = clk::now();
  sum->num_residual_blocks = (int64_t)h->nblocks_global;
  sum->reduced_dim = h->n_user;
  std::fill(g_launches, g_launches + kLfCount, (int64_t)0);
  auto finish = [&](int rc) {
    std::copy(g_launches, g_launches + kLfCount, h->last_launches);
    sum->time_total_s = std::chrono::duration<double>(clk::now() - t_begin).count();
    return rc;
  };
  if (h->local_ok) {
    const int rc = solve_local(h, sum);
    if (rc != kLocalRefused) return finish(rc);
  }

  launch_cam_scales(h->nc, h->d_cam_slot, h->d_cmask, h->d_diagU, 0, h->d_cs, s);
  launch_build_camtab(h->nc, h->d_q, h->d_t, h->d_intr, h->d_intr_idx, h->d_cs, h->d_camtab, s);
  if (h->n == 0 && h->nvarpts_global == 0.0) {
    double fx[3], c3[3];
    if (int rc = cost_of_records(h, true, fx)) return rc;
    double fixed = fx[0] + fx[1];
    if (int rc = allreduce_host(h, &fixed, 1)) return rc;
    sum->fixed_cost = fixed;
    if (int rc = cost_of_records(h, false, c3)) return rc;
    double c = c3[0] + c3[1];
    if (int rc = allreduce_host(h, &c, 1)) return rc;
    sum->initial_cost = sum->final_cost = c + fixed;
    sum->termination = MPSFM_TERM_NO_VARIABLES;
    return finish(0);
  }
  MPSFM_TRY(hipMemsetAsync(h->d_scal, 0, sizeof(double) * U_COUNT, s));
  launch_fixed_cost(h, h->d_scal + 12);
  if (int rc = prepare_scales(h)) return rc;
  if (h->np > 0) MPSFM_TRY(hipMemcpyAsync(h->d_pts2, h->d_pts, sizeof(double) * 3 * h->np, hipMemcpyDeviceToDevice, s));
  MPSFM_TRY(hipMemsetAsync(h->d_yc, 0, sizeof(double) * (size_t)std::max(h->n_user, 1), s));
  MPSFM_TRY(hipMemsetAsync(h->d_gc, 0, sizeof(double) * (size_t)std::max(h->n_user, 1), s));
  launch_cam_update(h->nc, h->d_cam_slot, h->d_q, h->d_t, h->d_cs, h->d_yc, h->d_gc, h->d_q2, h->d_t2, h->d_scal, s);
  const int nb = (int)std::min<int64_t>(1024, std::max<int64_t>(1, (h->np + kThreads - 1) / kThreads));
  launch_pts_sqnorm(h->np, h->rt.pt_kv, h->d_pts, h->d_costpart, nb, s);
  launch_reduce_cols(h->d_costpart, nb, 1, 1, 0u, h->d_scal + U_XN_SQ_PTS, s);

  h->h_ctl[0] = initial_ctl(o);
  MPSFM_TRY(hipMemcpyAsync(h->d_ctl, &h->h_ctl[0], sizeof(LmCtl), hipMemcpyHostToDevice, s));
  double* sums = nullptr;
  if (sharded(h)) {
    sums = h->d_costpart;
    launch_lm_pack(h->d_scal, sums, s);
    if (int rc = allreduce_dev(h, sums, 3)) return rc;
  }
  launch_lm_init(h->d_ctl, h->d_scal, sums, s);
  const LmOpts lo = lm_opts_of(o);
  const LmCtl* ctl = h->d_ctl;
  const double no_radius = 0.0;
  const bool fuse_prologue = [] { const char* e = std::getenv("MPSFM_FUSE_PROLOGUE"); return !(e && std::atoi(e) == 0); }();
  const bool fuse_cam = [] { const char* e = std::getenv("MPSFM_FUSE_CAM"); return !(e && std::atoi(e) == 0); }();
  const bool pt_handoff = pt_handoff_enabled() && h->d_pt_fac != nullptr;
  h->ov.entry_list = chol_entry_list();
  const bool fused_prologue = fuse_prologue && h->nlong == 0 && h->n_dense > 0 && h->n_dense == h->nchunks;
  auto enqueue_front = [&](int it) -> int {
    hipEvent_t* ev = (it & 1) ? h->ev2 : h->ev;
    MPSFM_TRY(hipEventRecord(ev[0], s));
    if (!fused_prologue)
      launch_lm_prologue(h->d_ctl, h->d_red, h->red_count, h->nc, h->np, h->d_q, h->d_t, h->d_camtab, h->d_pts, h->d_q2, h->d_t2, h->d_camtab2, h->d_pts2, s);
    if (int rc = run_track_sweep(h, no_radius, ctl, true, fused_prologue, pt_handoff)) return rc;
    if (int rc = allreduce_dev(h, h->d_red, h->red_count)) return rc;
    MPSFM_TRY(hipEventRecord(ev[1], s));
    return 0;
  };
  auto enqueue_back = [&](int it) -> int {
    hipEvent_t* ev = (it & 1) ? h->ev2 : h->ev;
    if (int rc = run_dense(h, no_radius, ctl)) return rc;
    MPSFM_TRY(hipEventRecord(ev[2], s));
    const bool fused_cam = fuse_cam && fused_prologue;
    CamUpdArgs cu{1, h->nc, h->d_cam_slot, h->d_cam_of_slot, h->d_q, h->d_t, h->d_cs, h->d_gc, h->d_intr, h->d_intr_idx,
                  h->d_q2, h->d_t2, h->d_camtab2, h->d_scal, h->d_fail};
    if (!fused_cam)
      launch_cam_update(h->nc, h->d_cam_slot, h->d_q, h->d_t, h->d_cs, h->d_yc, h->d_gc, h->d_q2, h->d_t2, h->d_scal, s,
                        h->d_intr, h->d_intr_idx, h->d_camtab2, h->d_fail, ctl);
    {
      SweepArgs a = sweep_args(h, no_radius, ctl);
      if (pt_handoff) a.pt_fac = h->d_pt_fac;
      launch_update_sweep(a, h->nchunks, s, fused_cam ? &cu : nullptr);
    }
    if (!sharded(h)) {
      launch_lm_reduce_decide(h->d_part, h->d_part2, h->nchunks + h->nlong, h->d_ctl, h->d_scal, lo, &h->h_ctl[it & 1], s);
    } else {
      if (h->nchunks + h->nlong > 0) launch_reduce_cols(h->d_part2, h->nchunks + h->nlong, 8, 5, 0u, h->d_scal, s);
      if (int rc = allreduce_dev(h, h->d_scal, 5)) return rc;
      launch_lm_decide(h->d_ctl, h->d_scal, lo, &h->h_ctl[it & 1], s, h->d_redsc);
    }
    MPSFM_TRY(hipEventRecord(ev[3], s));
    return 0;
  };
  auto enqueue_iteration = [&](int it) -> int {
    if (int rc = enqueue_front(it)) return rc;
    return enqueue_back(it);
  };
  LmCtl last = h->h_ctl[0];
  if (last.term == kLmRunning) {
    if (int rc = enqueue_iteration(1)) return rc;
    const bool speculate = [] { const char* e = std::getenv("MPSFM_LM_SPECULATE"); return !(e && std::atoi(e) == 0); }();
    const int force_split = [] { const char* e = std::getenv("MPSFM_LM_SPLIT"); return e ? (std::atoi(e) != 0 ? 1 : 0) : -1; }();
    const bool can_split = speculate && !sharded(h) && fused_prologue;
    for (int it = 1;; ++it) {
      const bool split = can_split && (force_split >= 0 ? force_split == 1 : h->split_front_s >= kSplitMinFront);
      if (speculate) { if (int rc = split ? enqueue_front(it + 1) : enqueue_iteration(it + 1)) return rc; }
      hipEvent_t* ev = (it & 1) ? h->ev2 : h->ev;
      MPSFM_TRY(hipEventSynchronize(ev[3]));
      MPSFM_TRY(hipGetLastError());
      float ms;
      MPSFM_TRY(hipEventElapsedTime(&ms, ev[0], ev[1])); sum->time_linearize_s += 1e-3 * ms;
      h->split_front_s = 1e-3 * ms;
      MPSFM_TRY(hipEventElapsedTime(&ms, ev[1], ev[2])); sum->time_dense_s += 1e-3 * ms;
      MPSFM_TRY(hipEventElapsedTime(&ms, ev[2], ev[3])); sum->time_update_s += 1e-3 * ms;
      last = h->h_ctl[it & 1];
      if (o.verbose > 0) print_iteration(it, last, last.fixed_cost);
      if (last.term != kLmRunning) break;
      if (!speculate) { if (int rc = enqueue_iteration(it + 1)) return rc; }
      else if (split) { if (int rc = enqueue_back(it + 1)) return rc; }
    }
    launch_lm_accept(h->d_ctl, h->nc, h->np, h->d_q, h->d_t, h->d_camtab, h->d_pts, h->d_q2, h->d_t2, h->d_camtab2, h->d_pts2, s);
    MPSFM_TRY(hipStreamSynchronize(s));
  }
  return finish(summary_from_ctl(h, last, sum));
}
}

using namespace mpsfm;

extern "C" {

int mpsfm_abi_version(void) { return MPSFM_ABI_VERSION; }
const char* mpsfm_last_error(void) { return g_err.c_str(); }

int mpsfm_device_count(void) {
  int n = 0;
  if (hipGetDeviceCount(&n) != hipSuccess) return 0;
  int good = 0;
  for (int i = 0; i < n; ++i) {
    hipDeviceProp_t p;
    if (hipGetDeviceProperties(&p, i) == hipSuccess && std::strncmp(p.gcnArchName, "gfx950", 6) == 0) ++good;
  }
  return good;
}

void mpsfm_ba_default_options(mpsfm_ba_options* o) {
  if (!o) return;
  std::memset(o, 0, sizeof(*o));
  o->max_num_iterations = 50;
  o->function_tolerance = 1e-6;
  o->gradient_tolerance = 1e-10;
  o->parameter_tolerance = 1e-8;
  o->initial_trust_region_radius = 1e4;
  o->max_trust_region_radius = 1e16;
// ... 97 lines not shown
```

### mpsfm_amd/csrc/common.h

```cpp
#pragma once
#include <hip/hip_runtime.h>
#include <stdint.h>
#include <float.h>
#include <math.h>

#include "../../include/mpsfm_hip.h"
#include "chol_plan.h"

namespace mpsfm {

#ifndef MPSFM_TILE_CAMS
#define MPSFM_TILE_CAMS 16
#endif
#ifndef MPSFM_ITEM_PAIRS
#define MPSFM_ITEM_PAIRS 64
#endif
#ifndef MPSFM_CAM_COPIES
#define MPSFM_CAM_COPIES 3
#endif
#ifndef MPSFM_ENT_STAGE
#define MPSFM_ENT_STAGE 1024
#endif
#ifndef MPSFM_OBS_MAX
#define MPSFM_OBS_MAX 252
#endif

typedef double v4d __attribute__((ext_vector_type(4)));
constexpr int kThreads = 256;
constexpr int kObsMax = MPSFM_OBS_MAX;
constexpr int kPtsMax = MPSFM_OBS_MAX / 2;
constexpr int kTileCams = MPSFM_TILE_CAMS;
#ifndef MPSFM_LOCAL_CAMS
#define MPSFM_LOCAL_CAMS 254
#endif
constexpr int kLocalCamsMax = MPSFM_LOCAL_CAMS;
static_assert(kLocalCamsMax < 255, "local camera indices are 8 bits, 0xff marks a constant camera");
constexpr int kPairGroup = 6;
constexpr int kItemPairs = MPSFM_ITEM_PAIRS;
constexpr int kEntStage = MPSFM_ENT_STAGE;
static_assert(kObsMax <= 256 && kPtsMax <= 128, "chunk-relative record / landmark indices are packed into 8 bits (rec_meta, pair entries)");
constexpr int kMaxDevices = 16;
constexpr int kWStride = 18;
constexpr int kCamRec = 24;


struct ChunkHdr {
  int32_t rec0, nrec;
  int32_t pt0, npt;
  int32_t cam0, ncam;
  int32_t blk0, nblk;
  int32_t ent0, nent;
  int32_t dense;
  int32_t slab0;
};
constexpr int kDenseCams = 16;
constexpr int kDensePts = 96;
__host__ __device__ inline int dense_pts_cap(int ncams, int by_cams) { return (!by_cams || ncams <= 6) ? kDensePts : (ncams <= 8 ? 64 : (ncams <= 12 ? 48 : 32)); }
__host__ __device__ inline int64_t slab_doubles(int ncam) { return (int64_t)(ncam * (ncam + 1) / 2) * 36 + (int64_t)ncam * 18; }

struct RedDest { int32_t kind; int32_t dst; int32_t s0, s1; };

struct LongHdr {
  int32_t rec0, nrec;
  int32_t pt;
  int32_t kv;
  int64_t w0;
};

constexpr uint32_t kRecHasReproj = 1u << 16;
constexpr uint32_t kRecHasDepth = 1u << 17;
constexpr uint32_t kLcamConst = 255;

struct LossParams {
  int32_t reproj_type;
  double reproj_a;
  double reproj_mag;
  int32_t depth_type;
};

constexpr int kMaxRankSlots = 64;
enum { SC_COST = 0, SC_BAD = 1, SC_GMAX_PTS = 2, SC_RANK0 = 8, SC_COUNT = 8 + kMaxRankSlots };

enum {
  U_CAND_COST = 0, U_BAD = 1, U_MCC = 2, U_STEP_SQ_PTS = 3, U_XN_SQ_PTS = 4,
  U_STEP_SQ_CAMS = 5, U_XN_SQ_CAMS = 6, U_GMAX_CAMS = 7, U_X_COST = 8, U_X_BAD = 9,
  U_GMAX_PTS = 10, U_CHOL_FAIL = 11, U_COUNT = 16
};

struct LmHead {
  double radius, decrease_factor, x_norm, cur_cost, fixed_cost, initial_cost;
  double last_x_cost, last_cand, last_rel, last_step_norm, last_mcc;
  int32_t term;
  int32_t iter, invalid_run, check_gradient, accepted, n_success, n_unsuccess, n_cost_evals, n_jac_evals, last_chol_fail, trace_len, pad_;
};
struct LmCtl : LmHead {
  double trace_cost[MPSFM_MAX_TRACE], trace_radius[MPSFM_MAX_TRACE];
  uint8_t trace_accepted[MPSFM_MAX_TRACE];
};
constexpr int32_t kLmRunning = -1, kLmNumericError = -2;
struct LmOpts {
  double function_tolerance, gradient_tolerance, parameter_tolerance, min_relative_decrease, max_radius, min_radius;
  int32_t max_iterations, max_invalid_steps;
};
__device__ inline bool lm_over(const LmCtl* c) { return c != nullptr && __hip_atomic_load(&c->term, __ATOMIC_RELAXED, __HIP_MEMORY_SCOPE_AGENT) != kLmRunning; }
__device__ inline double lm_radius_of(const LmCtl* c) { return __hip_atomic_load(&c->radius, __ATOMIC_RELAXED, __HIP_MEMORY_SCOPE_AGENT); }
#define MPSFM_CONST_AS __attribute__((address_space(4)))
template <typename T>
__device__ __forceinline__ T load_const(const T* p) { return *reinterpret_cast<const MPSFM_CONST_AS T*>(reinterpret_cast<uintptr_t>(p)); }
__device__ __forceinline__ int32_t lm_term_chain(const LmCtl* c) {
  return c != nullptr ? __hip_atomic_load(&c->term, __ATOMIC_RELAXED, __HIP_MEMORY_SCOPE_WORKGROUP) : kLmRunning;
}
__device__ __forceinline__ bool lm_over_chain(int32_t term) { asm volatile("" : "+v"(term)); return __builtin_amdgcn_readfirstlane(term) != kLmRunning; }
__device__ __forceinline__ int32_t lm_term_chain(const LmCtl* c, const void* readable) {
  return __hip_atomic_load(c != nullptr ? &c->term : static_cast<const int32_t*>(readable), __ATOMIC_RELAXED, __HIP_MEMORY_SCOPE_WORKGROUP);
}
__device__ __forceinline__ double lm_radius_chain(const LmCtl* c, double fallback) {
  return c != nullptr ? __hip_atomic_load(&c->radius, __ATOMIC_RELAXED, __HIP_MEMORY_SCOPE_WORKGROUP) : fallback;
}

__device__ __forceinline__ int32_t lm_accepted_chain(const LmCtl* c, const void* readable) {
  return __hip_atomic_load(c != nullptr ? &c->accepted : static_cast<const int32_t*>(readable), __ATOMIC_RELAXED, __HIP_MEMORY_SCOPE_WORKGROUP);
}
__device__ __forceinline__ double lm_radius_chain(const LmCtl* c, const void* readable, double fallback) {
  const double r = __hip_atomic_load(c != nullptr ? &c->radius : static_cast<const double*>(readable), __ATOMIC_RELAXED, __HIP_MEMORY_SCOPE_WORKGROUP);
  return c != nullptr ? r : fallback;
}

__host__ __device__ inline double fast_rcp(double x) {
#ifdef __HIP_DEVICE_COMPILE__
  double y = __builtin_amdgcn_rcp(x);
  y = fma(y, fma(-x, y, 1.0), y);
  return fma(y, fma(-x, y, 1.0), y);
#else
  return 1.0 / x;
#endif
}
__host__ __device__ inline void fast_sqrt_rsqrt(double x, double& s, double& r) {
#ifdef __HIP_DEVICE_COMPILE__
  const double y = __builtin_amdgcn_rsq(x);
  double g = x * y, h = 0.5 * y;
  double e = fma(-g, h, 0.5);
  g = fma(g, e, g); h = fma(h, e, h);
  e = fma(-g, h, 0.5);
// ... 87 lines not shown
  if (!(t22 > 0.0)) return false;
  fast_sqrt_rsqrt(t22, l22, i22);
  const double i10 = -l10 * i00 * i11;
  const double i21 = -l21 * i11 * i22;
  const double i20 = -(l20 * i00 + l21 * i10) * i22;
  F[0] = i00; F[1] = i10; F[2] = i11; F[3] = i20; F[4] = i21; F[5] = i22;
  return true;
}

__host__ __device__ inline void sym3_mul(const double* S, double v0, double v1, double v2, double* o) {
  o[0] = S[0] * v0 + S[1] * v1 + S[2] * v2;
  o[1] = S[1] * v0 + S[3] * v1 + S[4] * v2;
  o[2] = S[2] * v0 + S[4] * v1 + S[5] * v2;
}

__host__ __device__ inline int64_t ut_block(int64_t i, int64_t j, int64_t ncv) {
  return i * ncv - (i * (i - 1)) / 2 + (j - i);
}
struct BlockSky {
  const int32_t* first;
  const int64_t* start;
  const int32_t* index;
  int32_t ns;
};
constexpr int kIndexMaxSlots = 4096;
__host__ __device__ inline bool sky_has(const BlockSky& k, int64_t i, int64_t j) {
  return k.index ? k.index[j * k.ns + i] >= 0 : i >= k.first[j];
}
__host__ __device__ inline int64_t sky_block(const BlockSky& k, int64_t i, int64_t j) {
  return k.index ? (int64_t)k.index[j * k.ns + i] : k.start[j] + (i - k.first[j]);
}
__host__ __device__ inline int vec_index(const int32_t* col_slot, int g, int n) {
  if (g >= n) return -1;
  if (!col_slot) return g;
  const int cs = col_slot[g];
  return cs < 0 ? -1 : (cs >> 3) * 6 + (cs & 7);
}
__host__ __device__ inline int64_t lt_tile(int64_t ti, int64_t tj) { return ti * (ti + 1) / 2 + tj; }

struct SweepArgs {
  const ChunkHdr* chunks;
  const int32_t* chunk_cams;
  const int32_t* rec_cam;
  const uint32_t* rec_meta;
  const double* rec_xy;
  const double* rec_d;
  const double* rec_m;
  const double* rec_a;
  const int32_t* pt_rec_start;
  const uint16_t* pt_kv;
  const uint32_t* blk_desc;
  const int32_t* blk_ent_start;
  const uint32_t* ents;
  const double* camtab;
  const double* pts;
  const double* ps;
  LossParams loss;
  double radius, min_diag, max_diag;
  int32_t ncv;
  int32_t dbg;
  const LongHdr* lhdr;
  int32_t nlong, nchunks;
  const int32_t* cam_slot;
  double* wl;
  double* slab;
  int32_t chunk0;
  int32_t pad0_;
  BlockSky sky;
  double* Sblk;
  double* gc;
  double* wv;
  double* diagU;
  double* part;
  double* diagV;
  const double* yc;
  const double* camtab2;
  double* pts2;
  double* part2;
  const LmCtl* ctl;
  int32_t adopt_on, adopt_nc;
  double* pts_rw; double* q_rw; double* t_rw; double* camtab_rw;
  const double* q2; const double* t2;
  double* red; int64_t nred;
  double* pt_fac;
};
struct CamUpdArgs {
  int32_t fuse, nc;
  const int32_t* cam_slot;
  const int32_t* cam_of_slot;
  const double* q; const double* t; const double* cs; const double* gc;
  const double* intr; const int32_t* intr_idx;
  double* q2; double* t2; double* camtab2; double* scal; int* chol_fail;
};
__device__ inline bool lm_accepted(const LmCtl* c) { return c != nullptr && __hip_atomic_load(&c->accepted, __ATOMIC_RELAXED, __HIP_MEMORY_SCOPE_AGENT) != 0; }

struct CostArgs {
  int64_t nrec;
  const int32_t* rec_cam; const int32_t* rec_pt; const uint32_t* rec_meta; const double* rec_xy;
  const double* rec_d; const double* rec_m; const double* rec_a;
  const double* camtab; const double* pts;
  LossParams loss;
  double* part;
};

constexpr int kPanelWavesDefault = 4;
struct DenseOverlap {
  int nb = 0;
  bool big = true;
  bool overlap = true;
  bool no_level = false;
  bool no_inverse = false;
  int panel_waves = kPanelWavesDefault;
  bool entry_list = false;
  hipStream_t s2 = nullptr;
  hipEvent_t evF[4] = {nullptr, nullptr, nullptr, nullptr};
  hipEvent_t evB[4] = {nullptr, nullptr, nullptr, nullptr};
};

struct LevelPlanDev {
  bool valid = false, use_pinv = false;
  const CholItem* d_items = nullptr;
  const LevelHead* d_heads = nullptr;
  const int32_t* d_srcs = nullptr;
  const int32_t* d_rows = nullptr;
  const int32_t* d_struct_start = nullptr;
  const int32_t* d_struct_rows = nullptr;
  const int32_t* d_back_cols = nullptr;
  const int32_t* d_col_slot = nullptr;
  const int32_t* d_asm_tiles = nullptr;
  const uint8_t* d_tile_live = nullptr;
  int32_t n_asm = 0, nlevels = 0;
  const int32_t* h_launch_start = nullptr;
  const int32_t* h_back_start = nullptr;
};

struct AssembleArgs {
  BlockSky sky;
  const double* Sblk; const double* gc; const double* wv; const double* diagU;
  int32_t ncv, n, nt;
  double radius, min_diag, max_diag;
  double* A;
  double* Pinv;
  const int32_t* tile_list;
  int32_t n_list;
  const int32_t* col_slot;
  int32_t n_vec;
  double* y;
  const uint8_t* live;
  const LmCtl* ctl;
};


}
```

### mpsfm_amd/csrc/dense_chol.hip

```cpp
#include "../../include/mpsfm_hip_debug.h"
#include "common.h"
#include "ba_launch.h"
#include "dense_tile.h"
#include "dev_resources.h"

namespace mpsfm {

constexpr int kPlainMaxTiles = 64;

__device__ __forceinline__ void assemble_quad(const AssembleArgs& P, double lm_radius, int ti, int tj, int r0, int rstep, int c, double out[4]) {
  const int n = P.n;
  const int C = tj * kTile + c;
  const int ic = vec_index(P.col_slot, C, n);
  if (ti == P.nt) {
    const double rhs = (tj < P.nt && ic >= 0) ? P.wv[ic] - P.gc[ic] : 0.0;
#pragma unroll
    for (int k = 0; k < 4; ++k) out[k] = (r0 + k * rstep == 0) ? rhs : 0.0;
    return;
  }
  const int icv = ic >= 0 ? ic : 0;
  const int bc = icv / 6, b = icv - bc * 6;
  int ir[4];
#pragma unroll
  for (int k = 0; k < 4; ++k) ir[k] = vec_index(P.col_slot, ti * kTile + r0 + k * rstep, n);
// ... 250 lines not shown
    return;
  }
  if (wave != 0) return;
  double a[kTile];
#pragma unroll
  for (int c = 0; c < kTile; ++c) a[c] = sp[c];
  if (!skip) stacked_panel<0>(a, lane, s_P, ok);
  if (tr && lane == 0) tr[3] = wall_clock64();
  if (fail && !ok && lane == 0) atomicExch(fail, 1);
  if (dst) {
    double2* d2 = reinterpret_cast<double2*>(dst);
#pragma unroll
    for (int c = 0; c < kTile; c += 2) d2[c >> 1] = make_double2(a[c], a[c + 1]);
  }
  if (tr && lane == 0) tr[4] = wall_clock64();
}

__global__ __launch_bounds__(kStepThreads) void k_chol_step(double* A, double* LinvT, int nt, int j, int* fail, int dbg, int c0, int tk_max,
                                                            int mode, int panel_waves, long long* trace) {
  __shared__ double s_T[kTile][kTile + 1];
  __shared__ double s_X[kTile][kTile + 1];
  __shared__ __attribute__((aligned(16))) double s_Lt[kPanelLds];
  const int lane = threadIdx.x & 63, wave = threadIdx.x >> 6;
  const int mi = wave & 1, ni = wave >> 1;
  if (dbg & 16) return;
  const int tk = j + 1 + blockIdx.y, ti = j + 1 + blockIdx.x;
  if (ti < tk || tk >= nt || ti > nt || tk > tk_max) return;
  double* C = A + lt_tile(ti, tk) * kTileElems;
  if (tk != j + 1 || (mode & kStepBig)) {
    v4d acc;
    quad_load(C, kTile, lane, mi, ni, acc);
    if (!(dbg & 4))
      for (int c = c0; c <= j; ++c) {
        double a[8], b[8];
        quad_operand(A + lt_tile(ti, c) * kTileElems, lane, mi, a);
        quad_operand(A + lt_tile(tk, c) * kTileElems, lane, ni, b);
        quad_gemm_sub(a, b, acc);
      }
    quad_store(C, kTile, lane, mi, ni, acc);
    return;
  }
  const bool own_update = (j >= 0) && !(mode & kStepNoOwnUpdate) && !(dbg & 4);
  const bool diag = (ti == tk);
  long long* tr = trace ? trace + ((size_t)(j + 1) * 2) * 8 : nullptr;
  const bool trace_on = diag && tr != nullptr && wave == 0;
  MPSFM_STAMP(0);
  {
    v4d dacc, xacc;
    quad_load(A + lt_tile(tk, tk) * kTileElems, kTile, lane, mi, ni, dacc);
    if (!diag) quad_load(C, kTile, lane, mi, ni, xacc);
    if (own_update) {
      const double* Lk = A + lt_tile(tk, j) * kTileElems;
      double am[8], bn[8];
      quad_operand(Lk, lane, mi, am);
      quad_operand(Lk, lane, ni, bn);
      quad_gemm_sub(am, bn, dacc);
      if (!diag) {
        quad_operand(A + lt_tile(ti, j) * kTileElems, lane, mi, am);
        quad_gemm_sub(am, bn, xacc);
      }
    }
    quad_store(&s_T[0][0], kTile + 1, lane, mi, ni, dacc);
    if (diag) {
#pragma unroll
      for (int r = 0; r < 4; ++r) xacc[r] = (16 * mi + (lane >> 4) + 4 * r == 16 * ni + (lane & 15)) ? 1.0 : 0.0;
    }
    quad_store(&s_X[0][0], kTile + 1, lane, mi, ni, xacc);
  }
  MPSFM_STAMP(1);
  __syncthreads();
  panel_section(panel_waves, s_T, s_X, s_Lt, (dbg & 1) != 0, diag ? LinvT + (size_t)tk * kTileElems : C, nullptr, diag ? fail : nullptr,
                diag ? tr : nullptr);
}


struct LevelArgs {
  double* A; double* LinvT; double* Pinv;
  const CholItem* items; const int32_t* srcs; const int32_t* rows;
  const LevelHead* heads;
  int* fail; int32_t nt, dbg;
  const LmCtl* ctl;
  long long* trace;
  int32_t panel_waves;
};

typedef int32_t v16i __attribute__((ext_vector_type(16)));
static_assert(kInvRows <= kHeadRows, "a role's rows must fit its launch record");
constexpr int kHeadSrc0 = 2, kHeadRow0 = kHeadSrc0 + kInlineSrc, kHeadOver = kHeadRow0 + kHeadRows;
constexpr int kPanelBatch = 2;
constexpr int kTrailBatch = 4;

__device__ __forceinline__ int head_src(const v16i& w, const int32_t* srcs, int q) {
  if (q >= kInlineSrc) return srcs[(uint32_t)w[kHeadOver] + (uint32_t)(q - kInlineSrc)];
  int e = w[kHeadSrc0];
#pragma unroll
  for (int r = 1; r < kInlineSrc; ++r) e = (q == r) ? w[kHeadSrc0 + r] : e;
  return e;
}
struct PanelOps { double am[8], bn[8], ax[8]; };
struct TrailOps { double a[8], b[8]; };
__device__ __forceinline__ void panel_request(const double* A, int ti, int tk, int e, bool diag, int lane, int mi, int ni, PanelOps& o) {
  const int c = e & 0xffff;
  const double* Lk = A + lt_tile(tk, c) * kTileElems;
  quad_operand(Lk, lane, mi, o.am);
  quad_operand(Lk, lane, ni, o.bn);
  if (!diag && (e & kSrcX)) quad_operand(A + lt_tile(ti, c) * kTileElems, lane, mi, o.ax);
}
__device__ __forceinline__ void panel_apply(const PanelOps& o, int e, bool diag, v4d& dacc, v4d& xacc) {
  quad_gemm_sub(o.am, o.bn, dacc);
  if (!diag && (e & kSrcX)) quad_gemm_sub(o.ax, o.bn, xacc);
}
__device__ __forceinline__ void trail_request(const double* A, int ti, int tk, int c, int lane, int mi, int ni, TrailOps& o) {
  quad_operand(A + lt_tile(ti, c) * kTileElems, lane, mi, o.a);
  quad_operand(A + lt_tile(tk, c) * kTileElems, lane, ni, o.b);
}

constexpr int kStageTile = kTile * kLdsLd;
static_assert(kPanelLds >= 2 * kStageTile, "the first source of a panel item is staged in the panel's LDS buffer");
__device__ __forceinline__ void stage_fetch(const double* __restrict__ T, double2& p0, double2& p1) {
  p0 = reinterpret_cast<const double2*>(T)[threadIdx.x];
  p1 = reinterpret_cast<const double2*>(T)[threadIdx.x + kStepThreads];
}
__device__ __forceinline__ void stage_park(const double2& p0, const double2& p1, double* S) {
  const int r = threadIdx.x >> 4, c2 = threadIdx.x & 15;
  *reinterpret_cast<double2*>(S + r * kLdsLd + 2 * c2) = p0;
  *reinterpret_cast<double2*>(S + (r + 16) * kLdsLd + 2 * c2) = p1;
}
__device__ __forceinline__ void quad_operand_lds(const double* S, int lane, int b, double (&o)[8]) {
  const double2* p = reinterpret_cast<const double2*>(S + (16 * b + (lane & 15)) * kLdsLd + 8 * (lane >> 4));
#pragma unroll
  for (int s = 0; s < 4; ++s) { const double2 x = p[s]; o[2 * s] = x.x; o[2 * s + 1] = x.y; }
}

template <bool kList>
__global__ __launch_bounds__(kStepThreads) void k_chol_level(LevelArgs G) {
  __shared__ double s_T[kTile][kTile + 1];
  __shared__ double s_X[kTile][kTile + 1];
  __shared__ __attribute__((aligned(16))) double s_Lt[kPanelLds];
  __shared__ __attribute__((aligned(16))) double s_S1[kList ? 2 : 2 * kStageTile];
  const int lane = threadIdx.x & 63, wave = threadIdx.x >> 6;
  const int mi = wave & 1, ni = wave >> 1;
  double* A = G.A;
  int type, ti, tk, nsrc;
  int32_t term = kLmRunning;
  const bool has_ctl = !kList && G.ctl != nullptr;
  v16i w = {};
  const int32_t* src = nullptr;
  if constexpr (kList) {
    if (lm_over(G.ctl)) return;
    if (G.dbg & 16) return;
    const CholItem it = G.items[blockIdx.x];
    type = it.type; ti = it.ti; tk = it.tk; nsrc = it.nsrc;
    src = G.srcs + it.src;
    if (type == kItemRole) {
      if (G.dbg & 8) return;
      int irow[kInvRows];
#pragma unroll
      for (int r = 0; r < kInvRows; ++r) irow[r] = G.rows[it.aux + min(r, nsrc - 1)];
      inv_role(A, G.LinvT, G.Pinv, G.nt, ti, irow, nsrc, tk, kLmRunning, false, s_T, s_Lt);
      return;
    }
  } else {
    term = lm_term_chain(G.ctl, G.heads);
    w = load_const(reinterpret_cast<const v16i*>(G.heads + blockIdx.x));
    type = w[0] & 0xffff; ti = (uint32_t)w[0] >> 16; tk = w[1] & 0xffff; nsrc = (uint32_t)w[1] >> 16;
    if (G.dbg & 16) return;
    if ((G.dbg & 4) && type != kItemRole) nsrc = 0;
    if (type == kItemRole) {
      if (G.dbg & 8) return;
      int irow[kInvRows];
      irow[0] = w[kHeadRow0];
#pragma unroll
      for (int r = 1; r < kInvRows; ++r) irow[r] = r < nsrc ? w[kHeadRow0 + r] : irow[r - 1];
      inv_role(A, G.LinvT, G.Pinv, G.nt, ti, irow, nsrc, tk, term, has_ctl, s_T, s_Lt);
      return;
    }
  }
  double* C = A + lt_tile(ti, tk) * kTileElems;
  if (type == kItemTrail) {
    v4d acc;
    if constexpr (kList) quad_load(C, kTile, lane, mi, ni, acc);
    if (kList ? !(G.dbg & 4) : true) {
      if constexpr (kList) {
        for (int q = 0; q < nsrc; ++q) {
          const int c = src[q];
          double a[8], b[8];
          quad_operand(A + lt_tile(ti, c) * kTileElems, lane, mi, a);
          quad_operand(A + lt_tile(tk, c) * kTileElems, lane, ni, b);
          quad_gemm_sub(a, b, acc);
        }
      } else {
        TrailOps o[kTrailBatch], cur;
#pragma unroll
        for (int q = 0; q < kTrailBatch; ++q)
          if (q < nsrc) trail_request(A, ti, tk, w[kHeadSrc0 + q], lane, mi, ni, o[q]);
        if (nsrc > kTrailBatch) trail_request(A, ti, tk, head_src(w, G.srcs, kTrailBatch), lane, mi, ni, cur);
        quad_load(C, kTile, lane, mi, ni, acc);
#pragma unroll
        for (int q = 0; q < kTrailBatch; ++q)
          if (q < nsrc) quad_gemm_sub(o[q].a, o[q].b, acc);
        for (int q = kTrailBatch; q < nsrc; ++q) {
          TrailOps nxt;
          const bool more = q + 1 < nsrc;
          if (more) trail_request(A, ti, tk, head_src(w, G.srcs, q + 1), lane, mi, ni, nxt);
          quad_gemm_sub(cur.a, cur.b, acc);
          if (more) cur = nxt;
        }
      }
    }
    if (has_ctl && lm_over_chain(term)) return;
    quad_store(C, kTile, lane, mi, ni, acc);
    return;
  }
  const bool diag = (ti == tk);
  long long* tr = G.trace ? G.trace + ((size_t)tk * 2) * 8 : nullptr;
  const bool trace_on = diag && tr != nullptr && wave == 0;
  MPSFM_STAMP(0);
  {
    v4d dacc, xacc;
    const double* D = A + lt_tile(tk, tk) * kTileElems;
    if constexpr (kList) {
      quad_load(D, kTile, lane, mi, ni, dacc);
      if (!diag) quad_load(C, kTile, lane, mi, ni, xacc);
    }
    if (kList ? !(G.dbg & 4) : true) {
      if constexpr (kList) {
        for (int q = 0; q < nsrc; ++q) {
          const int e = src[q], c = e & 0xffff;
          const double* Lk = A + lt_tile(tk, c) * kTileElems;
          double am[8], bn[8];
          quad_operand(Lk, lane, mi, am);
          quad_operand(Lk, lane, ni, bn);
          quad_gemm_sub(am, bn, dacc);
          if (!diag && (e & kSrcX)) {
            quad_operand(A + lt_tile(ti, c) * kTileElems, lane, mi, am);
            quad_gemm_sub(am, bn, xacc);
          }
        }
      } else {
        static_assert(kPanelBatch == 2, "two staged sources, written out (an indexed array of pieces ends up in scratch)");
        const int e0 = w[kHeadSrc0], e1 = w[kHeadSrc0 + 1];
        const bool s0 = nsrc > 0, s1 = nsrc > 1, x0 = s0 && !diag && (e0 & kSrcX), x1 = s1 && !diag && (e1 & kSrcX);
        double2 k0a = {}, k0b = {}, x0a = {}, x0b = {}, k1a = {}, k1b = {}, x1a = {}, x1b = {};
        PanelOps cur;
        int e_cur = 0;
        if (s0) stage_fetch(A + lt_tile(tk, e0 & 0xffff) * kTileElems, k0a, k0b);
        if (x0) stage_fetch(A + lt_tile(ti, e0 & 0xffff) * kTileElems, x0a, x0b);
        if (s1) stage_fetch(A + lt_tile(tk, e1 & 0xffff) * kTileElems, k1a, k1b);
        if (x1) stage_fetch(A + lt_tile(ti, e1 & 0xffff) * kTileElems, x1a, x1b);
        if (nsrc > kPanelBatch) { e_cur = head_src(w, G.srcs, kPanelBatch); panel_request(A, ti, tk, e_cur, diag, lane, mi, ni, cur); }
        quad_load(D, kTile, lane, mi, ni, dacc);
        if (!diag) quad_load(C, kTile, lane, mi, ni, xacc);
        if (has_ctl && lm_over_chain(term)) return;
        if (s0) {
          stage_park(k0a, k0b, s_Lt);
          if (x0) stage_park(x0a, x0b, s_Lt + kStageTile);
          if (s1) stage_park(k1a, k1b, s_S1);
          if (x1) stage_park(x1a, x1b, s_S1 + kStageTile);
          __syncthreads();
          double am[8], bn[8];
          quad_operand_lds(s_Lt, lane, mi, am);
          quad_operand_lds(s_Lt, lane, ni, bn);
          quad_gemm_sub(am, bn, dacc);
          if (x0) {
            quad_operand_lds(s_Lt + kStageTile, lane, mi, am);
            quad_gemm_sub(am, bn, xacc);
          }
          if (s1) {
            quad_operand_lds(s_S1, lane, mi, am);
            quad_operand_lds(s_S1, lane, ni, bn);
            quad_gemm_sub(am, bn, dacc);
            if (x1) {
              quad_operand_lds(s_S1 + kStageTile, lane, mi, am);
              quad_gemm_sub(am, bn, xacc);
            }
          }
        }
        for (int q = kPanelBatch; q < nsrc; ++q) {
          PanelOps nxt;
          const bool more = q + 1 < nsrc;
          const int e_nxt = more ? head_src(w, G.srcs, q + 1) : 0;
          if (more) panel_request(A, ti, tk, e_nxt, diag, lane, mi, ni, nxt);
          panel_apply(cur, e_cur, diag, dacc, xacc);
          if (more) { cur = nxt; e_cur = e_nxt; }
        }
      }
    }
    quad_store(&s_T[0][0], kTile + 1, lane, mi, ni, dacc);
    if (diag) {
#pragma unroll
      for (int r = 0; r < 4; ++r) xacc[r] = (16 * mi + (lane >> 4) + 4 * r == 16 * ni + (lane & 15)) ? 1.0 : 0.0;
    }
    quad_store(&s_X[0][0], kTile + 1, lane, mi, ni, xacc);
  }
  MPSFM_STAMP(1);
  __syncthreads();
  panel_section(G.panel_waves, s_T, s_X, s_Lt, (G.dbg & 1) != 0, diag ? G.LinvT + (size_t)tk * kTileElems : C, nullptr, diag ? G.fail : nullptr,
                diag ? tr : nullptr);
}

__global__ __launch_bounds__(kStepThreads) void k_panel_probe(const double* dx, int waves, double* out, int* fail) {
  __shared__ double s_T[kTile][kTile + 1];
  __shared__ double s_X[kTile][kTile + 1];
  __shared__ __attribute__((aligned(16))) double s_Lt[kPanelLds];
  for (int e = threadIdx.x; e < kTileElems; e += kStepThreads) {
    s_T[e >> 5][e & 31] = dx[e];
    s_X[e >> 5][e & 31] = dx[kTileElems + e];
  }
  __syncthreads();
  panel_section(waves, s_T, s_X, s_Lt, false, out + kTileElems, out, fail, nullptr);
}
extern "C" int mpsfm_debug_panel_factor(const double* dx, int waves, double* out, int* ok) {
  if (!dx || !out || !ok || (waves != 1 && waves != kWgWaves)) return MPSFM_EINVAL;
  const size_t bytes = (size_t)2 * kTileElems * sizeof(double);
  DeviceBlocks own;
  double* d_in = own.alloc<double>((size_t)2 * kTileElems);
  double* d_out = own.alloc<double>((size_t)2 * kTileElems);
  int* d_fail = own.alloc<int>(1);
  hipError_t e = (d_in && d_out && d_fail) ? hipSuccess : hipErrorOutOfMemory;
  int h_fail = 0;
  if (e == hipSuccess) e = hipMemcpy(d_in, dx, bytes, hipMemcpyHostToDevice);
  if (e == hipSuccess) e = hipMemset(d_out, 0, bytes);
  if (e == hipSuccess) e = hipMemset(d_fail, 0, sizeof(int));
  if (e == hipSuccess) {
    hipLaunchKernelGGL(k_panel_probe, dim3(1), dim3(kStepThreads), 0, nullptr, d_in, waves, d_out, d_fail);
    e = hipGetLastError();
  }
  if (e == hipSuccess) e = hipMemcpy(out, d_out, bytes, hipMemcpyDeviceToHost);
  if (e == hipSuccess) e = hipMemcpy(&h_fail, d_fail, sizeof(int), hipMemcpyDeviceToHost);
  if (e != hipSuccess) return e == hipErrorOutOfMemory ? MPSFM_ENOMEM : MPSFM_EHIP;
  *ok = h_fail ? 0 : 1;
  return MPSFM_OK;
}

__global__ __launch_bounds__(256) void k_back_level(const double* A, const double* LinvT, const int32_t* cols, const int32_t* struct_start,
                                                    const int32_t* struct_rows, int nt, int n, double* ybuf, double* y, const int32_t* col_slot, const LmCtl* ctl) {
  __shared__ double s_part[8][kTile];
  __shared__ double s_v[kTile];
  const int32_t term = lm_term_chain(ctl);
  const int j = cols[blockIdx.x];
  const int c = threadIdx.x & 31, part = threadIdx.x >> 5;
  const int r0 = struct_start[j], r1 = struct_start[j + 1] - 1;
  double sacc = 0.0;
  for (int q = r0 + part; q < r1; q += 8) {
    const int i = struct_rows[q];
    const double* Tl = A + lt_tile(i, j) * kTileElems + c;
    const double* yi = ybuf + (size_t)i * kTile;
#pragma unroll 8
    for (int r = 0; r < kTile; ++r) sacc = __builtin_fma(Tl[r * kTile], yi[r], sacc);
  }
  if (lm_over_chain(term)) return;
  s_part[part][c] = sacc;
  __syncthreads();
  if (part == 0) {
    double v = A[lt_tile(nt, j) * kTileElems + c];
#pragma unroll
    for (int q = 0; q < 8; ++q) v -= s_part[q][c];
    s_v[c] = v;
  }
  __syncthreads();
  if (part == 0) {
    const double* Li = LinvT + (size_t)j * kTileElems + c * kTile;
    double yr = 0.0;
#pragma unroll
    for (int q = 0; q < kTile; ++q) yr = __builtin_fma(Li[q], s_v[q], yr);
    ybuf[(size_t)j * kTile + c] = yr;
    const int iy = vec_index(col_slot, j * kTile + c, n);
    if (iy >= 0) y[iy] = yr;
  }
}
// ... 96 lines not shown
  const int32_t term = lm_term_chain(ctl);
  const int k = blockIdx.x, sp = blockIdx.y, c = threadIdx.x & 31, part = threadIdx.x >> 5;
  const int first = k + 1 + sp;
  const int m = first < nt ? (nt - first + kInvSplit - 1) / kInvSplit : 0;
  const int own = sp == 0 ? 1 : 0;
  if (m + own == 0) return;
  for (int idx = threadIdx.x; idx < (m + own) * kTile; idx += 256) {
    const int slot = idx >> 5, r = idx & 31;
    const int i = (own && slot == 0) ? k : first + kInvSplit * (slot - own);
    const double* z = A + lt_tile(nt, i) * kTileElems;
    const double* Li = LinvT + (size_t)i * kTileElems + r * kTile;
    double sacc = 0.0;
#pragma unroll 8
    for (int q = 0; q < kTile; ++q) sacc = __builtin_fma(Li[q], z[q], sacc);
    s_w[idx] = sacc;
  }
  double pv[kInvPre][4];
#pragma unroll
  for (int j = 0; j < kInvPre; ++j)
    if (j < m) {
      const double* Pt = Pinv + lt_tile(first + kInvSplit * j, k) * kTileElems;
#pragma unroll
      for (int r = 0; r < 4; ++r) pv[j][r] = Pt[(4 * part + r) * kTile + c];
    }
  if (lm_over_chain(term)) return;
  __syncthreads();
  double sacc = 0.0;
#pragma unroll
  for (int j = 0; j < kInvPre; ++j)
    if (j < m) {
      const double* w = s_w + (j + own) * kTile;
#pragma unroll
      for (int r = 0; r < 4; ++r) sacc += pv[j][r] * w[4 * part + r];
    }
  for (int j = kInvPre; j < m; ++j) {
    const double* Pt = Pinv + lt_tile(first + kInvSplit * j, k) * kTileElems;
    const double* w = s_w + (j + own) * kTile;
#pragma unroll
    for (int r = 4 * part; r < 4 * part + 4; ++r) sacc += Pt[r * kTile + c] * w[r];
  }
  s_part[part][c] = sacc;
  __syncthreads();
  if (part == 0) {
    double v = 0.0;
#pragma unroll
    for (int q = 0; q < 8; ++q) v += s_part[q][c];
    const int g = k * kTile + c;
    const int iy = vec_index(col_slot, g, n);
    if (iy >= 0) atomicAdd(&y[iy], (own ? s_w[c] : 0.0) - v);
  }
}

void launch_assemble(const AssembleArgs& a, hipStream_t s) {
  const int64_t ntiles = a.tile_list ? (int64_t)a.n_list : (int64_t)(a.nt + 1) * (a.nt + 2) / 2;
  count_launch(kLfAssemble);
  hipLaunchKernelGGL(k_assemble, dim3((unsigned)ntiles), dim3(256), 0, s, a);
}

static void launch_big(double* A, int nt, int j, int c0, int tk_lo, int tk_hi, hipStream_t s) {
  if (tk_hi < tk_lo) return;
  const int rows = nt - tk_lo + 1, cols = tk_hi - tk_lo + 1;
  hipLaunchKernelGGL(k_big_update, dim3((rows + 1) / 2, (cols + 1) / 2), dim3(256), 0, s, A, nt, j, c0, tk_lo, tk_hi);
}

size_t dense_work_doubles(int nt) {
  const size_t t = (size_t)(nt > 0 ? nt : 1);
  size_t n = t * kTileElems + 2 * t * kTile + (t + 1) * kTileElems;
  if (nt <= kPlainMaxTiles) n += (t * (t + 1) / 2) * kTileElems;
  return n;
}
int dense_plain_max_tiles() { return kPlainMaxTiles; }
int dense_inv_rows() { return kInvRows; }
bool dense_level(const DenseOverlap* ov, const LevelPlanDev* lp) { return lp && lp->valid && !(ov && (ov->nb > 0 || ov->no_level)); }
static int dense_panel_width(int nt, const DenseOverlap* ov) {
  return (ov && ov->nb > 0) ? ov->nb : ((nt <= kPlainMaxTiles) ? nt : 8);
}
double* dense_pinv(double* work, int nt, const DenseOverlap* ov, const LevelPlanDev* lp) {
  if (nt <= 0 || nt > kPlainMaxTiles || (ov && (ov->no_inverse || ov->nb > 0))) return nullptr;
  if (dense_level(ov, lp) && !lp->use_pinv) return nullptr;
  return work + (size_t)nt * kTileElems + 2 * (size_t)nt * kTile + ((size_t)nt + 1) * kTileElems;
}

void launch_dense_solve(double* A, double* work, int nt, int n, double* y, int* fail, hipStream_t s, DenseOverlap* ov, const LevelPlanDev* lp,
                        const LmCtl* ctl) {
  if (nt <= 0) return;
  double* LinvT = work;
  double* zbuf = work + (size_t)nt * kTileElems;
  const int panel_waves = (ov ? ov->panel_waves : kPanelWavesDefault) == 1 ? 1 : kWgWaves;
  if (dense_level(ov, lp)) {
    double* Pinv = dense_pinv(work, nt, ov, lp);
    LevelArgs G{A, LinvT, Pinv, nullptr, lp->d_srcs, lp->d_rows, nullptr, fail, nt, g_dbg_flags, ctl, g_chol_trace, panel_waves};
    const bool list = ov && ov->entry_list;
    for (int l = 0; l < lp->nlevels; ++l) {
      const int grid = lp->h_launch_start[l + 1] - lp->h_launch_start[l];
      if (grid <= 0) continue;
      G.items = lp->d_items + lp->h_launch_start[l];
      G.heads = lp->d_heads + lp->h_launch_start[l];
      count_launch(kLfCholLevel);
      if (list) hipLaunchKernelGGL(k_chol_level<true>, dim3((unsigned)grid), dim3(kStepThreads), 0, s, G);
      else hipLaunchKernelGGL(k_chol_level<false>, dim3((unsigned)grid), dim3(kStepThreads), 0, s, G);
    }
    if (Pinv) {
      count_launch(kLfDenseRest);
      hipLaunchKernelGGL(k_inv_y, dim3(nt, kInvSplit), dim3(256), 0, s, A, LinvT, Pinv, nt, n, y, lp->d_col_slot, ctl);
      return;
    }
    for (int l = 0; l < lp->nlevels; ++l) {
      const int grid = lp->h_back_start[l + 1] - lp->h_back_start[l];
      if (grid <= 0) continue;
      count_launch(kLfDenseRest);
      hipLaunchKernelGGL(k_back_level, dim3((unsigned)grid), dim3(256), 0, s, A, LinvT, lp->d_back_cols + lp->h_back_start[l], lp->d_struct_start,
                         lp->d_struct_rows, nt, n, zbuf, y, lp->d_col_slot, ctl);
    }
    return;
  }
  const int NB = dense_panel_width(nt, ov);
  const bool big_kernel = !ov || ov->big;
  const bool overlap = ov && ov->s2 && ov->overlap && big_kernel && NB < nt;
  int npanel = 0;
  bool b_pending = false;
  for (int p0 = 0; p0 < nt; p0 += NB, ++npanel) {
    const int pend = (p0 + NB - 1 < nt - 1) ? p0 + NB - 1 : nt - 1;
    hipLaunchKernelGGL(k_chol_step, dim3(nt - p0 + 1, 1), dim3(kStepThreads), 0, s, A, LinvT, nt, p0 - 1, fail, g_dbg_flags, p0 - 1, p0,
                       kStepNoOwnUpdate, panel_waves, g_chol_trace);
    for (int j = p0; j <= pend - 1; ++j) {
      const int rows = nt - j, cols = pend - j;
      hipLaunchKernelGGL(k_chol_step, dim3(rows, cols), dim3(kStepThreads), 0, s, A, LinvT, nt, j, fail, g_dbg_flags, j, pend, 0, panel_waves, g_chol_trace);
    }
    if (pend >= nt - 1) break;
    if (!big_kernel) {
      hipLaunchKernelGGL(k_chol_step, dim3(nt - pend, nt - 1 - pend), dim3(kStepThreads), 0, s, A, LinvT, nt, pend, fail, g_dbg_flags, p0, nt - 1,
                         kStepBig, panel_waves, g_chol_trace);
    } else if (!overlap) {
      launch_big(A, nt, pend, p0, pend + 1, nt - 1, s);
    } else {
      const int qend = (pend + NB < nt - 1) ? pend + NB : nt - 1;
      hipEvent_t evF = ov->evF[npanel & 3], evB = ov->evB[npanel & 3];
      (void)hipEventRecord(evF, s);
      if (b_pending) (void)hipStreamWaitEvent(s, ov->evB[(npanel - 1) & 3], 0);
      launch_big(A, nt, pend, p0, pend + 1, qend, s);
      if (qend < nt - 1) {
        (void)hipStreamWaitEvent(ov->s2, evF, 0);
        launch_big(A, nt, pend, p0, qend + 1, nt - 1, ov->s2);
        (void)hipEventRecord(evB, ov->s2);
        b_pending = true;
      } else {
        b_pending = false;
      }
    }
  }
  if (overlap && npanel > 0) {
    for (int k = 0; k < 4; ++k) (void)hipStreamWaitEvent(s, ov->evB[k], 0);
  }
  hipLaunchKernelGGL(k_z_init, dim3((nt * kTile + 255) / 256), dim3(256), 0, s, A, nt, zbuf);
  for (int t1 = nt; t1 > 0; t1 -= kBsG) {
    const int t0 = t1 - kBsG > 0 ? t1 - kBsG : 0;
    hipLaunchKernelGGL(k_backsub_group, dim3(t0 > 0 ? t0 : 1), dim3(256), 0, s, A, LinvT, nt, n, t0, t1, zbuf, y, lp ? lp->d_col_slot : nullptr);
  }
}

}
```

### mpsfm_amd/csrc/sweep_dense.hip

```cpp
#include "sweep_dense_body.h"
#include "ba_launch.h"
#include <algorithm>

namespace mpsfm {

__global__ __launch_bounds__(kThreads, 3) void k_track_sweep_dense(SweepArgs A) {
  __shared__ DenseLds S;
  dense_sweep_chunk<false>(A, blockIdx.x + A.chunk0, A.radius, nullptr, S, A.part);
}

__global__ __launch_bounds__(256) void k_reduce_slabs(const RedDest* __restrict__ dests, int ndest, const int32_t* __restrict__ srcs,
                                                      const double* __restrict__ slab, double* Sblk, double* gc, double* wv, double* diagU,
                                                      const LmCtl* ctl) {
  if (lm_over(ctl)) return;
  const int w = blockIdx.x * 4 + (threadIdx.x >> 6), lane = threadIdx.x & 63;
  if (w >= ndest) return;
  const RedDest D = dests[w];
  bool active;
  if (D.kind == 2) active = lane < 18;
  else if (D.kind == 1) { const int ra = lane / 6, cb = lane - 6 * ra; active = lane < 36 && cb >= ra; }
  else active = lane < 36;
  double acc[8] = {0, 0, 0, 0, 0, 0, 0, 0};
  int s = D.s0;
  for (; s + 8 <= D.s1; s += 8) {
    int32_t o[8];
#pragma unroll
    for (int k = 0; k < 8; ++k) o[k] = srcs[s + k];
    if (active) {
#pragma unroll
      for (int k = 0; k < 8; ++k) acc[k] += slab[(size_t)o[k] * 18 + lane];
    }
  }
  for (int k = 0; s < D.s1; ++s, ++k)
    if (active) acc[k & 7] += slab[(size_t)srcs[s] * 18 + lane];
  const double v = ((acc[0] + acc[1]) + (acc[2] + acc[3])) + ((acc[4] + acc[5]) + (acc[6] + acc[7]));
  if (!active || v == 0.0) return;
  if (D.kind == 2) {
    double* base = lane < 6 ? gc : (lane < 12 ? wv : diagU);
    atomicAdd(&base[(size_t)D.dst * 6 + (lane % 6)], v);
  } else {
    atomicAdd(&Sblk[(size_t)D.dst * 36 + lane], v);
    if (D.kind == 1) {
    }
  }
}

void launch_track_sweep_dense(const SweepArgs& a, int nchunks, hipStream_t s) {
  if (nchunks > 0) { count_launch(kLfTrackSweep); hipLaunchKernelGGL(k_track_sweep_dense, dim3(nchunks), dim3(kThreads), 0, s, a); }
}
void launch_reduce_slabs(const RedDest* dests, int ndest, const int32_t* srcs, const double* slab, double* Sblk, double* gc, double* wv, double* diagU,
                         const LmCtl* ctl, hipStream_t s) {
  if (ndest > 0) { count_launch(kLfReduceSlabs); hipLaunchKernelGGL(k_reduce_slabs, dim3((ndest + 3) / 4), dim3(256), 0, s, dests, ndest, srcs, slab, Sblk, gc, wv, diagU, ctl); }
}

}
```

### mpsfm_amd/csrc/sweep_dense_body.h

```cpp
#pragma once
#include "common.h"
#include "sweep_common.h"

namespace mpsfm {

namespace {
constexpr int kAccU = 2 * kDenseCams * 21;
constexpr int kAccG = 2 * kDenseCams * 6;

}

template <int NT>
__device__ __forceinline__ void schur_units(double* s_W, const uint8_t* s_rec, const double* s_U, double* slab, int tid, int npt, int ncam,
                                            int ncopy, int cstride, int dbg) {
  constexpr int NP = NT * (NT + 1) / 2;
  const int lane = tid & 63, wave = tid >> 6;
  const int rc = lane & 15, kq = lane >> 4;
  int camt[NT], a3t[NT];
  bool camv[NT];
#pragma unroll
  for (int t = 0; t < NT; ++t) {
    const int r = 16 * t + rc;
    camt[t] = r / 6; a3t[t] = (r - 6 * (r / 6)) * 3;
    camv[t] = camt[t] < ncam; camt[t] = camv[t] ? camt[t] : 0;
// ... 145 lines not shown
      rec_request(g2, rnxt);
#pragma unroll
      for (int c = 0; c < 3; ++c)
#pragma unroll
        for (int j = 0; j < NP; ++j)
          acc[j][c & 1] = __builtin_amdgcn_mfma_f64_16x16x4f64(x[2 * j][c], x[2 * j + 1][c], acc[j][c & 1], 0, 0, 0);
      row_fix(rcur, xn);
#pragma unroll
      for (int o = 0; o < NO; ++o)
#pragma unroll
        for (int c = 0; c < 3; ++c) x[o][c] = xn[o][c];
    }
  }
  if (!(dbg & 4)) {
#pragma unroll
    for (int j = 0; j < NP; ++j) {
#pragma unroll
      for (int r = 0; r < 4; ++r) {
        const int row = 16 * pti[j] + kq + 4 * r, col = 16 * ptj[j] + rc;
        const int ci = row / 6, cj = col / 6;
        const int ra = row - 6 * ci, cb = col - 6 * cj;
        if (cj < ncam && (ci < cj || (ci == cj && ra <= cb))) {
          double v = -(acc[j][0][r] + acc[j][1][r]);
          if (ci == cj) {
            const int u = ra * 6 - (ra * (ra - 1)) / 2 + (cb - ra);
            double uu = 0.0;
            for (int q = 0; q < ncopy; ++q) uu += s_U[(q * cstride + ci) * 21 + u];
            v += uu;
          }
          slab[(cj * (cj + 1) / 2 + ci) * 36 + ra * 6 + cb] = v;
        }
      }
    }
  }
}


struct __attribute__((aligned(16))) DenseLds {
  double W[kObsMax * kWStride];
  double V[kDensePts * 6];
  double g[kDensePts * 3];
  double U[kAccU];
  double gc[kAccG];
  double wv[kAccG];
  uint8_t rec[kDensePts * kDenseCams] __attribute__((aligned(4)));
  int32_t slot[kDenseCams];
  double red[3 * (kThreads / 64)];
};
static_assert(kObsMax <= 254, "record indices in DenseLds::rec are 8 bits, 255 marks an empty cell");
static_assert(sizeof(DenseLds) <= 54608, "three workgroups per CU need at most 160 KiB / 3 of LDS each");

template <bool kLocal>
__device__ __forceinline__ void dense_sweep_chunk(const SweepArgs& A, int cix, double lm_radius, const double* l_tab, DenseLds& S, double* part) {
  const int tid = thread_index<kLocal>();
  long long* const trace = (A.dbg & 128) && (tid & 63) == 0 ? reinterpret_cast<long long*>(A.diagV) + ((size_t)cix * 4 + (tid >> 6)) * 16 : nullptr;
#define MPSFM_STAMP(k) do { if (trace) trace[k] = (long long)clock64(); } while (0)
  MPSFM_STAMP(0);
  if (trace) trace[12] = (long long)wall_clock64();
  const ChunkHdr H = A.chunks[cix];
  [[maybe_unused]] int32_t term = kLmRunning, accepted = 0;
  if constexpr (!kLocal) {
    term = lm_term_chain(A.ctl, A.chunks);
    accepted = lm_accepted_chain(A.ctl, A.chunks);
    lm_radius = lm_radius_chain(A.ctl, A.chunks, lm_radius);
  }
  const int nrec = H.nrec, npt = H.npt, ncam = H.ncam;
  const int ncopy = ncam <= 8 ? 4 : 2, cstride = ncam <= 8 ? 8 : 16;
  const bool has_rec = tid < nrec;
  uint32_t my_meta = *(has_rec ? &A.rec_meta[H.rec0 + tid] : reinterpret_cast<const uint32_t*>(A.chunks));
  int cam = *(has_rec ? &A.rec_cam[H.rec0 + tid] : reinterpret_cast<const int32_t*>(A.chunks));
  double2 xy = *(has_rec ? &reinterpret_cast<const double2*>(A.rec_xy)[H.rec0 + tid] : reinterpret_cast<const double2*>(A.chunks));
  [[maybe_unused]] int32_t my_slot = 0;
  if constexpr (kLocal) my_slot = *(tid < ncam ? &A.chunk_cams[H.cam0 + tid] : reinterpret_cast<const int32_t*>(A.chunks));
  if constexpr (!kLocal) {
    if (A.ctl != nullptr && lm_over_chain(term)) return;
  }

  bool adopt = false;
  if constexpr (!kLocal) {
    if (A.adopt_on) {
      adopt = A.ctl != nullptr && __builtin_amdgcn_readfirstlane(accepted) != 0;
      const int64_t g0 = (int64_t)(cix - A.chunk0) * kThreads + tid, gstep = (int64_t)A.nchunks * kThreads;
      for (int64_t e = g0; e < A.nred; e += gstep) A.red[e] = 0.0;
      if (adopt) {
        for (int i = tid; i < 3 * npt; i += kThreads) A.pts_rw[(size_t)3 * H.pt0 + i] = A.pts2[(size_t)3 * H.pt0 + i];
        const int64_t n_q = 4 * (int64_t)A.adopt_nc, n_t = 3 * (int64_t)A.adopt_nc, n_tab = (int64_t)kCamRec * A.adopt_nc;
        for (int64_t e = g0; e < n_q + n_t + n_tab; e += gstep) {
          if (e < n_q) A.q_rw[e] = A.q2[e];
          else if (e < n_q + n_t) A.t_rw[e - n_q] = A.t2[e - n_q];
          else A.camtab_rw[e - n_q - n_t] = A.camtab2[e - n_q - n_t];
        }
      }
    }
  }
  const double* const pts_at = adopt ? A.pts2 : A.pts;
  const double* const camtab_at = adopt ? A.camtab2 : A.camtab;
  for (int i = tid; i < npt * 6; i += kThreads) S.V[i] = 0.0;
  for (int i = tid; i < npt * 3; i += kThreads) S.g[i] = 0.0;
  for (int i = tid; i < kAccU; i += kThreads) S.U[i] = 0.0;
  for (int i = tid; i < kAccG; i += kThreads) { S.gc[i] = 0.0; S.wv[i] = 0.0; }
  for (int i = tid; i < npt * (kDenseCams / 4); i += kThreads) reinterpret_cast<uint32_t*>(S.rec)[i] = 0xffffffffu;
  if constexpr (kLocal) { if (tid < ncam) S.slot[tid] = my_slot; }
  MPSFM_STAMP(1);
  __syncthreads();
  MPSFM_STAMP(2);
  asm volatile("" : "+v"(my_meta), "+v"(cam));
  if (!has_rec) my_meta = 0;

  double my_cost = 0.0;
  int my_bad = 0;
  uint16_t my_kv = 0xffff;
  double my_ps[3] = {0, 0, 0};
  double my_w[18];
#pragma unroll
  for (int i = 0; i < 18; ++i) my_w[i] = 0.0;
  double Vg[9] = {0, 0, 0, 0, 0, 0, 0, 0, 0};
  if (tid < nrec) {
    const uint32_t meta = my_meta;
    const int lcam = meta & 0xff;
    const int lpt = (meta >> 8) & 0xff;
    const int pix = H.pt0 + lpt;
    const double X[3] = {pts_at[3 * pix], pts_at[3 * pix + 1], pts_at[3 * pix + 2]};
    const double psc[3] = {A.ps[3 * pix], A.ps[3 * pix + 1], A.ps[3 * pix + 2]};
    my_kv = A.pt_kv[pix];
    double d = 1.0, m = 0.0, a = 1.0;
    if (meta & kRecHasDepth) { const int rix = H.rec0 + tid; d = A.rec_d[rix]; m = A.rec_m[rix]; a = A.rec_a[rix]; }
    my_ps[0] = psc[0]; my_ps[1] = psc[1]; my_ps[2] = psc[2];
    RecLin L;
    if (trace) { asm volatile("s_waitcnt vmcnt(0)" ::: "memory"); trace[10] = (long long)clock64(); }
    linearize_record(camera_row<kLocal>(camtab_at, l_tab, S.slot, cam, lcam), X, psc, meta, xy.x, xy.y, d, m, a, A.loss, L);
    my_cost = L.cost;
    if (trace) { asm volatile("" : "+v"(L.Jc[0]), "+v"(L.Jp[8]), "+v"(L.cost)); trace[11] = (long long)clock64(); }
    my_bad = L.ok ? 0 : 1;
    if (L.ok) {
      if (psc[0] != 0.0) {
#pragma unroll
        for (int r = 0; r < 3; ++r) {
          const double j0 = L.Jp[3 * r], j1 = L.Jp[3 * r + 1], j2 = L.Jp[3 * r + 2];
          Vg[0] += j0 * j0; Vg[1] += j0 * j1; Vg[2] += j0 * j2; Vg[3] += j1 * j1; Vg[4] += j1 * j2; Vg[5] += j2 * j2;
          Vg[6] += j0 * L.r[r]; Vg[7] += j1 * L.r[r]; Vg[8] += j2 * L.r[r];
        }
      }
      if (lcam != (int)kLcamConst && !(A.dbg & 1)) {
        const int acc = (lpt % ncopy) * cstride + lcam;
        int u = 0;
#pragma unroll
        for (int i = 0; i < 6; ++i) {
          const double gci = L.Jc[i] * L.r[0] + L.Jc[6 + i] * L.r[1] + L.Jc[12 + i] * L.r[2];
          atomicAdd(&S.gc[acc * 6 + i], gci);
#pragma unroll
          for (int j = i; j < 6; ++j, ++u) {
            const double uij = L.Jc[i] * L.Jc[j] + L.Jc[6 + i] * L.Jc[6 + j] + L.Jc[12 + i] * L.Jc[12 + j];
            atomicAdd(&S.U[acc * 21 + u], uij);
          }
        }
#pragma unroll
        for (int i = 0; i < 6; ++i)
#pragma unroll
          for (int j = 0; j < 3; ++j)
            my_w[i * 3 + j] = L.Jc[i] * L.Jp[j] + L.Jc[6 + i] * L.Jp[3 + j] + L.Jc[12 + i] * L.Jp[6 + j];
      }
    }
  }
  {
    const int my_lpt = (int)((my_meta >> 8) & 0xff);
    seg_step<1>(my_lpt, Vg); seg_step<2>(my_lpt, Vg); seg_step<4>(my_lpt, Vg); seg_step<8>(my_lpt, Vg);
// ... 120 lines not shown
```

Before: 9.857 billion residual-block evals/s.

## Scatter reduced Schur blocks directly into dense front tiles and fuse damping into first Cholesky level

Result: faster. 10.00 billion residual-block evals/s, median of 6 (+1.5%).

```diff
diff --git a/include/mpsfm_hip_debug.h b/include/mpsfm_hip_debug.h
--- a/include/mpsfm_hip_debug.h
+++ b/include/mpsfm_hip_debug.h
@@ -22,6 +22,8 @@
 int mpsfm_debug_graph_union(const uint8_t* adj, int32_t world, int32_t n, uint8_t* out);
 
 int mpsfm_debug_pt_handoff(mpsfm_ba_handle* h);
+int mpsfm_debug_direct_front(mpsfm_ba_handle* h);
+int mpsfm_debug_direct_assemble(mpsfm_ba_handle* h, double radius, double* A_parent, double* A_direct, double* damp, uint8_t* live, int64_t info[4]);
 int mpsfm_debug_dense_solve_given(mpsfm_ba_handle* h, const double* S, const double* rhs, int32_t n, int32_t* failed);
 int mpsfm_debug_read_trace(mpsfm_ba_handle* h, long long* out, int64_t count);
 int64_t mpsfm_debug_table(mpsfm_ba_handle* h, int32_t which, void* out, int64_t cap);
diff --git a/mpsfm_amd/abi.py b/mpsfm_amd/abi.py
--- a/mpsfm_amd/abi.py
+++ b/mpsfm_amd/abi.py
@@ -421,6 +421,8 @@
     "mpsfm_debug_run_parts": (I64, [I32, I32]),
     "mpsfm_debug_graph_union": (C.c_int, [P, I32, I32, P]),
     "mpsfm_debug_pt_handoff": (C.c_int, [P]),
+    "mpsfm_debug_direct_front": (C.c_int, [P]),
+    "mpsfm_debug_direct_assemble": (C.c_int, [P, C.c_double, P, P, P, P, P]),
     "mpsfm_debug_dense_solve_given": (C.c_int, [P, P, P, I32, C.POINTER(I32)]),
     "mpsfm_debug_read_trace": (C.c_int, [P, P, I64]),
     "mpsfm_debug_table": (I64, [P, I32, P, I64]),
diff --git a/mpsfm_amd/capi.py b/mpsfm_amd/capi.py
--- a/mpsfm_amd/capi.py
+++ b/mpsfm_amd/capi.py
@@ -143,6 +143,18 @@
 
     def pt_handoff(self) -> bool:
         return bool(lib().mpsfm_debug_pt_handoff(self._h))
+
+    def direct_front(self) -> bool:
+        return bool(lib().mpsfm_debug_direct_front(self._h))
+
+    def direct_assemble(self, radius: float = 1e4) -> dict:
+        nt = self.dense_plan()["tile_columns"]
+        ntiles = (nt + 1) * (nt + 2) // 2
+        ap, ad = np.zeros((ntiles, 32, 32)), np.zeros((ntiles, 32, 32))
+        damp, live, info = np.zeros(32 * nt), np.zeros(ntiles, np.uint8), np.zeros(4, np.int64)
+        _check(lib().mpsfm_debug_direct_assemble(self._h, float(radius), ap.ctypes.data, ad.ctypes.data, damp.ctypes.data, live.ctypes.data, info.ctypes.data))
+        assert int(info[0]) == nt
+        return dict(parent=ap, direct=ad, damp=damp, live=live.astype(bool), nt=nt, n=int(info[1]), n_live=int(info[2]), unzeroed=int(info[3]))
 
     def sweep_once(self, radius: float = 1e4) -> float:
         ms = C.c_float(0)
diff --git a/mpsfm_amd/csrc/ba_build.hip b/mpsfm_amd/csrc/ba_build.hip
--- a/mpsfm_amd/csrc/ba_build.hip
+++ b/mpsfm_amd/csrc/ba_build.hip
@@ -54,10 +54,34 @@
   std::vector<uint8_t> live((size_t)(PL.nt + 1) * (size_t)(PL.nt + 2) / 2, 0);
   for (int32_t id : PL.asm_tiles) live[(size_t)id] = 1;
   LevelPlanDev& D = h->lp;
+  std::vector<int32_t> pinv_tiles;
+  std::vector<uint8_t> level0((size_t)std::max(PL.nt, 1), 0);
+  bool first_is_plain = false;
+  {
+    std::vector<uint8_t> seen(live.size(), 0);
+    for (const CholItem& it : PL.items)
+      if (it.type == kItemRole)
+        for (uint32_t q = 0; q < it.nsrc; ++q) {
+          const int64_t id = lt_tile(PL.rows[(size_t)it.aux + q], it.tk);
+          if (!seen[(size_t)id]) { seen[(size_t)id] = 1; pinv_tiles.push_back((int32_t)id); }
+        }
+    std::sort(pinv_tiles.begin(), pinv_tiles.end());
+    for (int l = 0; l + 1 < (int)PL.launch_start.size(); ++l) {
+      if (PL.launch_start[(size_t)l + 1] <= PL.launch_start[(size_t)l]) continue;
+      first_is_plain = true;
+      for (int32_t i = PL.launch_start[(size_t)l]; i < PL.launch_start[(size_t)l + 1]; ++i) {
+        const CholItem& it = PL.items[(size_t)i];
+        if (it.type != kItemPanel || it.nsrc != 0) first_is_plain = false;
+        else if (it.ti == it.tk) level0[it.tk] = 1;
+      }
+      break;
+    }
+  }
   if (int rc = own.upload(&D.d_items, PL.items, &D.d_heads, PL.heads, &D.d_srcs, PL.srcs, &D.d_rows, PL.rows, &D.d_struct_start, PL.struct_start,
                           &D.d_struct_rows, PL.struct_rows, &D.d_back_cols, PL.back_cols, &D.d_asm_tiles, PL.asm_tiles,
-                          &D.d_col_slot, PL.slot_of_col, &D.d_tile_live, live))
+                          &D.d_col_slot, PL.slot_of_col, &D.d_tile_live, live, &D.d_pinv_tiles, pinv_tiles, &D.d_level0, level0))
     return rc;
+  D.n_pinv_tiles = (int32_t)pinv_tiles.size(); D.damp_in_launch0 = first_is_plain;
   if (PL.slot_of_col.empty()) D.d_col_slot = nullptr;
   level_plan_flags(PL, D);
   D.n_asm = (int32_t)PL.asm_tiles.size(); D.nlevels = PL.nlevels;
@@ -201,6 +225,8 @@
   if ((rc = own.alloc(&h->d_yc, (size_t)std::max(h->n_user, 1)))) return rc;
   if ((rc = own.alloc(&h->d_fail, 1))) return rc;
   MPSFM_TRY(hipMemsetAsync(h->d_fail, 0, sizeof(int), h->stream));
+  if (double* pinv = dense_pinv(h->d_dwork, h->nt, nullptr, nullptr))
+    MPSFM_TRY(hipMemsetAsync(pinv, 0, sizeof(double) * (size_t)h->nt * (size_t)(h->nt + 1) / 2 * 1024, h->stream));
   for (auto& e : h->ev) MPSFM_TRY(own.event(&e, true));
   opt.apply_dense(h->nt, h->plan, h->ov);
   if (h->nt > 64 || h->ov.nb > 0) {
@@ -220,6 +246,44 @@
   MPSFM_TRY(hipMemsetAsync(h->d_ps, 0, nps * 3 * sizeof(double), h->stream));
   MPSFM_TRY(hipMemsetAsync(h->d_yc, 0, (size_t)std::max(h->n_user, 1) * sizeof(double), h->stream));
   MPSFM_TRY(hipStreamSynchronize(h->stream));
+  return 0;
+}
+
+__global__ __launch_bounds__(256) void k_dest_cols(const RedDest* __restrict__ dests, int ndest, const RedCols* __restrict__ blk_cols,
+                                                   const int32_t* __restrict__ col_of_slot, RedDestCols* __restrict__ out) {
+  const int w = blockIdx.x * 256 + threadIdx.x;
+  if (w >= ndest) return;
+  const RedDest D = dests[w];
+  out[w] = RedDestCols{D, D.kind == 2 ? RedCols{col_of_slot[D.dst], 0} : blk_cols[D.dst], {0, 0}};
+}
+static int build_direct_tables(mpsfm_ba_handle* h) {
+  if (sharded(h) || h->nlong != 0 || h->n_dense <= 0 || h->n_dense != h->nchunks || !h->lp.valid || !h->lp.damp_in_launch0 || h->n <= 0 || h->n_red_dests <= 0)
+    return 0;
+  const CholPlan& PL = h->plan;
+  std::vector<int32_t> col((size_t)std::max(h->ncv, 1), 0);
+  for (int i = 0; i < h->ncv; ++i) col[(size_t)i] = PL.col_of_slot.empty() ? 6 * i : PL.col_of_slot[(size_t)i];
+  const BlockSky sky{h->spat.sky_first.data(), h->spat.sky_start.data(), h->spat.sky_index.empty() ? nullptr : h->spat.sky_index.data(), h->ncv};
+  std::vector<RedCols> blk_cols((size_t)std::max<int64_t>(h->spat.nblk, 1), RedCols{0, 0});
+  for (int j = 0; j < h->ncv; ++j)
+    for (int i = sky.index ? 0 : sky.first[j]; i <= j; ++i) {
+      if (!sky_has(sky, i, j)) continue;
+      const int64_t b = sky_block(sky, i, j);
+      if (b < 0 || b >= h->spat.nblk || col[(size_t)i] + 6 > h->n || col[(size_t)j] + 6 > h->n) return fail(MPSFM_EUNSUPPORTED, "internal: block index and plan disagree");
+      blk_cols[(size_t)b] = RedCols{col[(size_t)i], col[(size_t)j]};
+    }
+  RedCols* d_blk_cols = nullptr;
+  int32_t* d_col = nullptr;
+  DeviceBlocks& own = h->own;
+  if (int rc = own.upload(&d_blk_cols, blk_cols, &d_col, col)) return rc;
+  if (int rc = staged_drain()) return rc;
+  RedDestCols* out = nullptr;
+  if (int rc = own.alloc(&out, (size_t)h->n_red_dests)) return rc;
+  if (int rc = own.alloc(&h->d_diag_col, (size_t)h->nt * 32)) return rc;
+  hipLaunchKernelGGL(k_dest_cols, dim3((h->n_red_dests + 255) / 256), dim3(256), 0, h->stream, h->d_red_dests, h->n_red_dests, d_blk_cols, d_col, out);
+  MPSFM_TRY(hipGetLastError());
+  MPSFM_TRY(hipStreamSynchronize(h->stream));
+  own.drop(d_blk_cols); own.drop(d_col);
+  h->d_red_cols = out;
   return 0;
 }
 
@@ -333,6 +397,8 @@
   lap("upload tables");
   if (int rc = alloc_work_buffers(h, opt)) return rc;
   lap("allocate work buffers");
+  if (int rc = build_direct_tables(h)) return rc;
+  lap("direct assembly tables");
   return 0;
 }
 
diff --git a/mpsfm_amd/csrc/ba_debug.hip b/mpsfm_amd/csrc/ba_debug.hip
--- a/mpsfm_amd/csrc/ba_debug.hip
+++ b/mpsfm_amd/csrc/ba_debug.hip
@@ -1,6 +1,7 @@
 #include <algorithm>
 #include <atomic>
 #include <cstring>
+#include <limits>
 #include <vector>
 
 #include "../../include/mpsfm_hip_debug.h"
@@ -76,6 +77,62 @@
 }
 
 int mpsfm_debug_pt_handoff(mpsfm_ba_handle* h) { return h && h->d_pt_fac != nullptr ? 1 : 0; }
+
+int mpsfm_debug_direct_front(mpsfm_ba_handle* h) {
+  return h && direct_front(h) ? 1 : 0;
+}
+
+int mpsfm_debug_direct_assemble(mpsfm_ba_handle* h, double radius, double* A_parent, double* A_direct, double* damp, uint8_t* live, int64_t info[4]) {
+  if (!h || !A_parent || !A_direct || !damp || !live || !info) return fail(MPSFM_EINVAL, "handle or output is NULL");
+  if (!mpsfm_debug_direct_front(h)) return fail(MPSFM_EUNSUPPORTED, "the handle does not take the direct form of the front");
+  MPSFM_TRY(hipSetDevice(h->device));
+  if (!h->scales_ready) if (int rc = prepare_scales(h)) return rc;
+  hipStream_t s = h->stream;
+  const int nt = h->nt;
+  const size_t ntiles = (size_t)(nt + 1) * (size_t)(nt + 2) / 2;
+  const double nan = std::numeric_limits<double>::quiet_NaN();
+  std::vector<double> img(ntiles * 1024, 0.0);
+  std::fill(live, live + ntiles, (uint8_t)0);
+  for (int32_t id : h->plan.asm_tiles) { live[(size_t)id] = 1; std::fill(img.begin() + (size_t)id * 1024, img.begin() + ((size_t)id + 1) * 1024, nan); }
+  MPSFM_TRY(hipMemcpyAsync(h->d_A, img.data(), sizeof(double) * img.size(), hipMemcpyHostToDevice, s));
+  if (int rc = run_track_sweep(h, radius)) return rc;
+  run_assemble(h, radius);
+  MPSFM_TRY(hipMemcpyAsync(A_parent, h->d_A, sizeof(double) * img.size(), hipMemcpyDeviceToHost, s));
+  MPSFM_TRY(hipStreamSynchronize(s));
+  SweepArgs a = sweep_args(h, radius);
+  a.adopt_on = 1; a.adopt_nc = h->nc;
+  direct_zero_args(h, a);
+  MPSFM_TRY(hipMemcpyAsync(h->d_A, img.data(), sizeof(double) * img.size(), hipMemcpyHostToDevice, s));
+  for (int k = 0; k < 2; ++k) MPSFM_TRY(hipMemsetAsync(a.zero_p[k], 0xff, sizeof(double) * (size_t)a.zero_n[k], s));
+  const size_t npinv = (size_t)nt * (size_t)(nt + 1) / 2 * 1024;
+  std::vector<double> pimg(npinv, 0.0);
+  for (const CholItem& it : h->plan.items)
+    if (it.type == kItemRole)
+      for (uint32_t q = 0; q < it.nsrc; ++q) {
+        const size_t id = (size_t)lt_tile(h->plan.rows[(size_t)it.aux + q], it.tk);
+        std::fill(pimg.begin() + id * 1024, pimg.begin() + (id + 1) * 1024, nan);
+      }
+  MPSFM_TRY(hipMemcpyAsync(a.zero_P, pimg.data(), sizeof(double) * npinv, hipMemcpyHostToDevice, s));
+  launch_track_sweep_dense(a, h->n_dense, s);
+  const DirectAsm da = direct_asm(h);
+  launch_reduce_slabs(h->d_red_dests, h->n_red_dests, h->d_red_srcs, h->d_slab, h->d_Sblk, h->d_gc, h->d_wv, h->d_diagU, nullptr, s, &da);
+  std::vector<double> pinv(npinv), y((size_t)std::max(h->n_user, 1)), dcol((size_t)nt * 32);
+  MPSFM_TRY(hipMemcpyAsync(A_direct, h->d_A, sizeof(double) * img.size(), hipMemcpyDeviceToHost, s));
+  MPSFM_TRY(hipMemcpyAsync(pinv.data(), a.zero_P, sizeof(double) * pinv.size(), hipMemcpyDeviceToHost, s));
+  MPSFM_TRY(hipMemcpyAsync(y.data(), h->d_yc, sizeof(double) * (size_t)h->n_user, hipMemcpyDeviceToHost, s));
+  MPSFM_TRY(hipMemcpyAsync(dcol.data(), h->d_diag_col, sizeof(double) * dcol.size(), hipMemcpyDeviceToHost, s));
+  MPSFM_TRY(hipStreamSynchronize(s));
+  MPSFM_TRY(hipGetLastError());
+  h->last_radius = radius;
+  const int32_t* slot_of_col = h->plan.slot_of_col.empty() ? nullptr : h->plan.slot_of_col.data();
+  for (int g = 0; g < nt * 32; ++g)
+    damp[g] = vec_index(slot_of_col, g, h->n) < 0 ? -1.0 : std::min(std::max(dcol[(size_t)g], h->opt.min_lm_diagonal), h->opt.max_lm_diagonal) / radius;
+  int64_t bad = 0;
+  for (double v : pinv) bad += v == 0.0 ? 0 : 1;
+  for (int i = 0; i < h->n_user; ++i) bad += y[(size_t)i] == 0.0 ? 0 : 1;
+  info[0] = nt; info[1] = h->n; info[2] = (int64_t)h->plan.asm_tiles.size(); info[3] = bad;
+  return 0;
+}
 
 int mpsfm_ba_sweep_once(mpsfm_ba_handle* h, double radius, float* elapsed_ms) {
   if (!h) return fail(MPSFM_EINVAL, "handle is NULL");
diff --git a/mpsfm_amd/csrc/ba_handle.h b/mpsfm_amd/csrc/ba_handle.h
--- a/mpsfm_amd/csrc/ba_handle.h
+++ b/mpsfm_amd/csrc/ba_handle.h
@@ -32,6 +32,8 @@
   double* d_slab = nullptr;
   mpsfm::RedDest* d_red_dests = nullptr;
   int32_t* d_red_srcs = nullptr;
+  mpsfm::RedDestCols* d_red_cols = nullptr;
+  double* d_diag_col = nullptr;
   int n_red_dests = 0;
   int64_t n_red_srcs = 0, n_chunk_cams = 0, n_blk_desc = 0, n_blk_ent_start = 0, n_ents = 0;
   bool built_on_device = false;
@@ -109,9 +111,13 @@
 
 SweepArgs sweep_args(mpsfm_ba_handle* h, double radius, const LmCtl* ctl = nullptr);
 int prepare_scales(mpsfm_ba_handle* h);
-int run_track_sweep(mpsfm_ba_handle* h, double radius, const LmCtl* ctl = nullptr, bool in_loop = false, bool adopt = false, bool handoff = false);
+int run_track_sweep(mpsfm_ba_handle* h, double radius, const LmCtl* ctl = nullptr, bool in_loop = false, bool adopt = false, bool handoff = false,
+                    bool direct = false);
 void run_assemble(mpsfm_ba_handle* h, double radius, const LmCtl* ctl = nullptr);
-int run_dense(mpsfm_ba_handle* h, double radius, const LmCtl* ctl = nullptr);
+int run_dense(mpsfm_ba_handle* h, double radius, const LmCtl* ctl = nullptr, bool direct = false);
+bool direct_front(mpsfm_ba_handle* h);
+DirectAsm direct_asm(const mpsfm_ba_handle* h);
+void direct_zero_args(mpsfm_ba_handle* h, SweepArgs& a);
 bool chol_entry_list();
 
 struct LocalSkew { int32_t chunk = 0, mask = 0; int64_t ticks = 0; };
diff --git a/mpsfm_amd/csrc/ba_launch.h b/mpsfm_amd/csrc/ba_launch.h
--- a/mpsfm_amd/csrc/ba_launch.h
+++ b/mpsfm_amd/csrc/ba_launch.h
@@ -22,7 +22,7 @@
 void launch_update_sweep(const SweepArgs&, int nchunks, hipStream_t, const CamUpdArgs* cu = nullptr);
 void launch_track_sweep_dense(const SweepArgs&, int nchunks, hipStream_t);
 void launch_reduce_slabs(const RedDest* dests, int ndest, const int32_t* srcs, const double* slab, double* Sblk, double* gc, double* wv, double* diagU,
-                         const LmCtl* ctl, hipStream_t);
+                         const LmCtl* ctl, hipStream_t, const DirectAsm* direct = nullptr);
 void launch_cost_records(const CostArgs&, int nblocks, hipStream_t);
 void launch_reduce_cols(const double* part, int64_t rows, int stride, int ncols, uint32_t max_mask, double* out, hipStream_t,
                         double* out2 = nullptr, int gmax_slot = -1);
@@ -50,7 +50,7 @@
 extern int g_dbg_flags;
 void launch_assemble(const AssembleArgs&, hipStream_t);
 void launch_dense_solve(double* A, double* work, int nt, int n, double* y, int* fail, hipStream_t, DenseOverlap* ov, const LevelPlanDev* lp,
-                        const LmCtl* ctl = nullptr);
+                        const LmCtl* ctl = nullptr, const DampArgs* damp = nullptr);
 bool dense_level(const DenseOverlap* ov, const LevelPlanDev* lp);
 int dense_plain_max_tiles();
 int dense_inv_rows();
diff --git a/mpsfm_amd/csrc/ba_solver.hip b/mpsfm_amd/csrc/ba_solver.hip
--- a/mpsfm_amd/csrc/ba_solver.hip
+++ b/mpsfm_amd/csrc/ba_solver.hip
@@ -69,14 +69,31 @@
   return 0;
 }
 
-static void launch_sweeps(mpsfm_ba_handle* h, SweepArgs a, hipStream_t s) {
+static void launch_sweeps(mpsfm_ba_handle* h, SweepArgs a, hipStream_t s, bool direct) {
   launch_track_sweep_dense(a, h->n_dense, s);
-  launch_reduce_slabs(h->d_red_dests, h->n_red_dests, h->d_red_srcs, h->d_slab, h->d_Sblk, h->d_gc, h->d_wv, h->d_diagU, a.ctl, s);
+  const DirectAsm da = direct ? direct_asm(h) : DirectAsm{};
+  launch_reduce_slabs(h->d_red_dests, h->n_red_dests, h->d_red_srcs, h->d_slab, h->d_Sblk, h->d_gc, h->d_wv, h->d_diagU, a.ctl, s, direct ? &da : nullptr);
   a.chunk0 = h->n_dense;
   launch_track_sweep(a, h->nchunks - h->n_dense, false, s);
 }
 
-int run_track_sweep(mpsfm_ba_handle* h, double radius, const LmCtl* ctl, bool in_loop, bool adopt, bool handoff) {
+bool direct_front(mpsfm_ba_handle* h) {
+  const char* e = std::getenv("MPSFM_ASSEMBLE");
+  if (e && std::strcmp(e, "launch") == 0) return false;
+  const char* f = std::getenv("MPSFM_FUSE_PROLOGUE");
+  if (f && std::atoi(f) == 0) return false;
+  return h->d_red_cols != nullptr && !sharded(h) && h->n > 0 && dense_level(&h->ov, &h->lp) && dense_pinv(h->d_dwork, h->nt, &h->ov, &h->lp) != nullptr;
+}
+DirectAsm direct_asm(const mpsfm_ba_handle* h) { return DirectAsm{h->d_red_cols, h->d_A, h->d_diag_col, h->nt}; }
+void direct_zero_args(mpsfm_ba_handle* h, SweepArgs& a) {
+  a.red = h->d_gc; a.nred = h->red_count - h->sblk_count;
+  a.zero_p[0] = h->d_yc; a.zero_n[0] = h->n_user;
+  a.zero_p[1] = h->d_diag_col; a.zero_n[1] = (int64_t)h->nt * 32;
+  a.zero_A = h->d_A; a.zero_tiles = h->lp.d_asm_tiles; a.zero_ntiles = h->lp.n_asm;
+  a.zero_P = dense_pinv(h->d_dwork, h->nt, &h->ov, &h->lp); a.zero_ptiles = h->lp.d_pinv_tiles; a.zero_nptiles = h->lp.n_pinv_tiles;
+}
+
+int run_track_sweep(mpsfm_ba_handle* h, double radius, const LmCtl* ctl, bool in_loop, bool adopt, bool handoff, bool direct) {
   hipStream_t s = h->stream;
   if (!in_loop) launch_zero(h->d_red, h->red_count, ctl, s);
   SweepArgs a = sweep_args(h, radius, ctl);
@@ -84,9 +101,10 @@
     a.adopt_on = 1; a.adopt_nc = h->nc;
     a.pts_rw = h->d_pts; a.q_rw = h->d_q; a.t_rw = h->d_t; a.camtab_rw = h->d_camtab; a.q2 = h->d_q2; a.t2 = h->d_t2;
     a.red = h->d_red; a.nred = h->red_count;
+    if (direct) direct_zero_args(h, a);
   }
   if (handoff) a.pt_fac = h->d_pt_fac;
-  launch_sweeps(h, a, s);
+  launch_sweeps(h, a, s, direct && adopt);
   if (h->nchunks + h->nlong > 0 && !(in_loop && !sharded(h)))
     launch_reduce_cols(h->d_part, h->nchunks + h->nlong, 4, 3, 1u << 2, h->d_redsc, s, sharded(h) ? nullptr : h->d_scal + U_X_COST,
                        sharded(h) ? (h->opt.rank > 0 ? h->opt.rank : 0) % kMaxRankSlots : -1);
@@ -105,10 +123,11 @@
   launch_assemble(as, h->stream);
 }
 
-int run_dense(mpsfm_ba_handle* h, double radius, const LmCtl* ctl) {
+int run_dense(mpsfm_ba_handle* h, double radius, const LmCtl* ctl, bool direct) {
   if (h->n > 0) {
-    run_assemble(h, radius, ctl);
-    launch_dense_solve(h->d_A, h->d_dwork, h->nt, h->n, h->d_yc, h->d_fail, h->stream, &h->ov, &h->lp, ctl);
+    if (!direct) run_assemble(h, radius, ctl);
+    const DampArgs damp{h->d_diag_col, h->lp.d_col_slot, h->lp.d_level0, h->n, h->opt.min_lm_diagonal, h->opt.max_lm_diagonal, radius};
+    launch_dense_solve(h->d_A, h->d_dwork, h->nt, h->n, h->d_yc, h->d_fail, h->stream, &h->ov, &h->lp, ctl, direct ? &damp : nullptr);
   }
   return 0;
 }
@@ -270,19 +289,20 @@
   const bool pt_handoff = pt_handoff_enabled() && h->d_pt_fac != nullptr;
   h->ov.entry_list = chol_entry_list();
   const bool fused_prologue = fuse_prologue && h->nlong == 0 && h->n_dense > 0 && h->n_dense == h->nchunks;
+  const bool direct = fused_prologue && direct_front(h);
   auto enqueue_front = [&](int it) -> int {
     hipEvent_t* ev = (it & 1) ? h->ev2 : h->ev;
     MPSFM_TRY(hipEventRecord(ev[0], s));
     if (!fused_prologue)
       launch_lm_prologue(h->d_ctl, h->d_red, h->red_count, h->nc, h->np, h->d_q, h->d_t, h->d_camtab, h->d_pts, h->d_q2, h->d_t2, h->d_camtab2, h->d_pts2, s);
-    if (int rc = run_track_sweep(h, no_radius, ctl, true, fused_prologue, pt_handoff)) return rc;
+    if (int rc = run_track_sweep(h, no_radius, ctl, true, fused_prologue, pt_handoff, direct)) return rc;
     if (int rc = allreduce_dev(h, h->d_red, h->red_count)) return rc;
     MPSFM_TRY(hipEventRecord(ev[1], s));
     return 0;
   };
   auto enqueue_back = [&](int it) -> int {
     hipEvent_t* ev = (it & 1) ? h->ev2 : h->ev;
-    if (int rc = run_dense(h, no_radius, ctl)) return rc;
+    if (int rc = run_dense(h, no_radius, ctl, direct)) return rc;
     MPSFM_TRY(hipEventRecord(ev[2], s));
     const bool fused_cam = fuse_cam && fused_prologue;
     CamUpdArgs cu{1, h->nc, h->d_cam_slot, h->d_cam_of_slot, h->d_q, h->d_t, h->d_cs, h->d_gc, h->d_intr, h->d_intr_idx,
diff --git a/mpsfm_amd/csrc/common.h b/mpsfm_amd/csrc/common.h
--- a/mpsfm_amd/csrc/common.h
+++ b/mpsfm_amd/csrc/common.h
@@ -59,6 +59,8 @@
 __host__ __device__ inline int64_t slab_doubles(int ncam) { return (int64_t)(ncam * (ncam + 1) / 2) * 36 + (int64_t)ncam * 18; }
 
 struct RedDest { int32_t kind; int32_t dst; int32_t s0, s1; };
+struct RedCols { int32_t c0, c1; };
+struct alignas(32) RedDestCols { RedDest d; RedCols c; int32_t pad_[2]; };
 
 struct LongHdr {
   int32_t rec0, nrec;
@@ -312,6 +314,9 @@
   double* pts_rw; double* q_rw; double* t_rw; double* camtab_rw;
   const double* q2; const double* t2;
   double* red; int64_t nred;
+  double* zero_p[2]; int64_t zero_n[2];
+  double* zero_A; const int32_t* zero_tiles; int32_t zero_ntiles;
+  double* zero_P; const int32_t* zero_ptiles; int32_t zero_nptiles;
   double* pt_fac;
 };
 struct CamUpdArgs {
@@ -359,9 +364,27 @@
   const int32_t* d_col_slot = nullptr;
   const int32_t* d_asm_tiles = nullptr;
   const uint8_t* d_tile_live = nullptr;
+  const int32_t* d_pinv_tiles = nullptr;
+  int32_t n_pinv_tiles = 0;
+  const uint8_t* d_level0 = nullptr;
+  bool damp_in_launch0 = false;
   int32_t n_asm = 0, nlevels = 0;
   const int32_t* h_launch_start = nullptr;
   const int32_t* h_back_start = nullptr;
+};
+
+struct DirectAsm {
+  const RedDestCols* dests;
+  double* A;
+  double* diag_col;
+  int32_t nt;
+};
+struct DampArgs {
+  const double* diag_col;
+  const int32_t* col_slot;
+  const uint8_t* level0;
+  int32_t n;
+  double min_diag, max_diag, radius;
 };
 
 struct AssembleArgs {
diff --git a/mpsfm_amd/csrc/dense_chol.hip b/mpsfm_amd/csrc/dense_chol.hip
--- a/mpsfm_amd/csrc/dense_chol.hip
+++ b/mpsfm_amd/csrc/dense_chol.hip
@@ -356,7 +356,38 @@
   const LmCtl* ctl;
   long long* trace;
   int32_t panel_waves;
+  DampArgs damp;
+  int32_t nitems;
 };
+
+struct DampReq { double du, radius; int32_t cs; };
+__device__ __forceinline__ void damp_request(const DampArgs& P, const LmCtl* ctl, int g, DampReq& q) {
+  q.du = P.diag_col[g];
+  const int32_t cs = *(P.col_slot ? P.col_slot + min(g, P.n - 1) : reinterpret_cast<const int32_t*>(P.diag_col));
+  q.radius = lm_radius_chain(ctl, P.diag_col, P.radius);
+  q.cs = g >= P.n ? -1 : (P.col_slot ? cs : 0);
+}
+__device__ __forceinline__ double damp_value(const DampArgs& P, const DampReq& q, double d) {
+  return q.cs < 0 ? 1.0 : d + fmin(fmax(q.du, P.min_diag), P.max_diag) / q.radius;
+}
+__device__ __forceinline__ void damp_apply(const DampArgs& P, const DampReq& q, int mi, int ni, int lane, v4d& dacc) {
+  if (mi != ni || ((lane & 15) & 3) != (lane >> 4)) return;
+#pragma unroll
+  for (int r = 0; r < 4; ++r)
+    if (r == ((lane & 15) >> 2)) dacc[r] = damp_value(P, q, dacc[r]);
+}
+__device__ __forceinline__ void damp_columns(const DampArgs& P, const LmCtl* ctl, double* A, int nt, int g) {
+  const int32_t term = lm_term_chain(ctl, P.diag_col);
+  const bool mine = g < nt * kTile;
+  const int gc = mine ? g : 0, tk = gc >> 5, c = gc & 31;
+  const uint8_t in_panel = P.level0[tk];
+  double* d = A + lt_tile(tk, tk) * kTileElems + c * kTile + c;
+  const double v = *d;
+  DampReq q;
+  damp_request(P, ctl, gc, q);
+  if (ctl != nullptr && lm_over_chain(term)) return;
+  if (mine && !in_panel) *d = damp_value(P, q, v);
+}
 
 typedef int32_t v16i __attribute__((ext_vector_type(16)));
 static_assert(kInvRows <= kHeadRows, "a role's rows must fit its launch record");
@@ -406,7 +437,7 @@
   for (int s = 0; s < 4; ++s) { const double2 x = p[s]; o[2 * s] = x.x; o[2 * s + 1] = x.y; }
 }
 
-template <bool kList>
+template <bool kList, bool kDamp>
 __global__ __launch_bounds__(kStepThreads) void k_chol_level(LevelArgs G) {
   __shared__ double s_T[kTile][kTile + 1];
   __shared__ double s_X[kTile][kTile + 1];
@@ -415,6 +446,12 @@
   const int lane = threadIdx.x & 63, wave = threadIdx.x >> 6;
   const int mi = wave & 1, ni = wave >> 1;
   double* A = G.A;
+  if constexpr (kDamp) {
+    if ((int)blockIdx.x >= G.nitems) {
+      damp_columns(G.damp, G.ctl, A, G.nt, ((int)blockIdx.x - G.nitems) * kStepThreads + (int)threadIdx.x);
+      return;
+    }
+  }
   int type, ti, tk, nsrc;
   int32_t term = kLmRunning;
   const bool has_ctl = !kList && G.ctl != nullptr;
@@ -493,6 +530,8 @@
   {
     v4d dacc, xacc;
     const double* D = A + lt_tile(tk, tk) * kTileElems;
+    [[maybe_unused]] DampReq dq;
+    if constexpr (kDamp) damp_request(G.damp, G.ctl, tk * kTile + 16 * ni + (lane & 15), dq);
     if constexpr (kList) {
       quad_load(D, kTile, lane, mi, ni, dacc);
       if (!diag) quad_load(C, kTile, lane, mi, ni, xacc);
@@ -560,6 +599,7 @@
         }
       }
     }
+    if constexpr (kDamp) damp_apply(G.damp, dq, mi, ni, lane, dacc);
     quad_store(&s_T[0][0], kTile + 1, lane, mi, ni, dacc);
     if (diag) {
 #pragma unroll
@@ -822,23 +862,32 @@
 }
 
 void launch_dense_solve(double* A, double* work, int nt, int n, double* y, int* fail, hipStream_t s, DenseOverlap* ov, const LevelPlanDev* lp,
-                        const LmCtl* ctl) {
+                        const LmCtl* ctl, const DampArgs* damp) {
   if (nt <= 0) return;
   double* LinvT = work;
   double* zbuf = work + (size_t)nt * kTileElems;
   const int panel_waves = (ov ? ov->panel_waves : kPanelWavesDefault) == 1 ? 1 : kWgWaves;
   if (dense_level(ov, lp)) {
     double* Pinv = dense_pinv(work, nt, ov, lp);
-    LevelArgs G{A, LinvT, Pinv, nullptr, lp->d_srcs, lp->d_rows, nullptr, fail, nt, g_dbg_flags, ctl, g_chol_trace, panel_waves};
+    LevelArgs G{A, LinvT, Pinv, nullptr, lp->d_srcs, lp->d_rows, nullptr, fail, nt, g_dbg_flags, ctl, g_chol_trace, panel_waves, damp ? *damp : DampArgs{}, 0};
     const bool list = ov && ov->entry_list;
+    bool damped = damp == nullptr;
     for (int l = 0; l < lp->nlevels; ++l) {
       const int grid = lp->h_launch_start[l + 1] - lp->h_launch_start[l];
       if (grid <= 0) continue;
       G.items = lp->d_items + lp->h_launch_start[l];
       G.heads = lp->d_heads + lp->h_launch_start[l];
       count_launch(kLfCholLevel);
-      if (list) hipLaunchKernelGGL(k_chol_level<true>, dim3((unsigned)grid), dim3(kStepThreads), 0, s, G);
-      else hipLaunchKernelGGL(k_chol_level<false>, dim3((unsigned)grid), dim3(kStepThreads), 0, s, G);
+      if (!damped) {
+        G.nitems = grid;
+        const unsigned g2 = (unsigned)(grid + (nt * kTile + kStepThreads - 1) / kStepThreads);
+        if (list) hipLaunchKernelGGL((k_chol_level<true, true>), dim3(g2), dim3(kStepThreads), 0, s, G);
+        else hipLaunchKernelGGL((k_chol_level<false, true>), dim3(g2), dim3(kStepThreads), 0, s, G);
+        damped = true;
+        continue;
+      }
+      if (list) hipLaunchKernelGGL((k_chol_level<true, false>), dim3((unsigned)grid), dim3(kStepThreads), 0, s, G);
+      else hipLaunchKernelGGL((k_chol_level<false, false>), dim3((unsigned)grid), dim3(kStepThreads), 0, s, G);
     }
     if (Pinv) {
       count_launch(kLfDenseRest);
diff --git a/mpsfm_amd/csrc/sweep_dense.hip b/mpsfm_amd/csrc/sweep_dense.hip
--- a/mpsfm_amd/csrc/sweep_dense.hip
+++ b/mpsfm_amd/csrc/sweep_dense.hip
@@ -9,17 +9,35 @@
   dense_sweep_chunk<false>(A, blockIdx.x + A.chunk0, A.radius, nullptr, S, A.part);
 }
 
-__global__ __launch_bounds__(256) void k_reduce_slabs(const RedDest* __restrict__ dests, int ndest, const int32_t* __restrict__ srcs,
+template <bool kDirect>
+__global__ __launch_bounds__(256, kDirect ? 8 : 1) void k_reduce_slabs(const RedDest* __restrict__ dests, int ndest, const int32_t* __restrict__ srcs,
                                                       const double* __restrict__ slab, double* Sblk, double* gc, double* wv, double* diagU,
-                                                      const LmCtl* ctl) {
+                                                      const LmCtl* ctl, DirectAsm T) {
   if (lm_over(ctl)) return;
   const int w = blockIdx.x * 4 + (threadIdx.x >> 6), lane = threadIdx.x & 63;
   if (w >= ndest) return;
-  const RedDest D = dests[w];
+  RedDest D;
+  [[maybe_unused]] RedCols cc{0, 0};
+  if constexpr (kDirect) { const RedDestCols X = T.dests[w]; D = X.d; cc = X.c; }
+  else D = dests[w];
   bool active;
   if (D.kind == 2) active = lane < 18;
   else if (D.kind == 1) { const int ra = lane / 6, cb = lane - 6 * ra; active = lane < 36 && cb >= ra; }
   else active = lane < 36;
+  [[maybe_unused]] int32_t o0 = 0, o1 = -1, col = 0;
+  if constexpr (kDirect) {
+    if (D.kind == 2) {
+      col = cc.c0 + lane % 6;
+      o0 = (int32_t)lt_tile(T.nt, col >> 5) * 1024 + (col & 31);
+    } else {
+      const int a = lane / 6, b = lane - 6 * a;
+      const int r = cc.c0 + a, c = cc.c1 + b;
+      const int R = r > c ? r : c, C = r > c ? c : r;
+      const int32_t id = active ? (int32_t)lt_tile(R >> 5, C >> 5) : 0;
+      o0 = id * 1024 + (R & 31) * 32 + (C & 31);
+      if ((R >> 5) == (C >> 5) && R != C) o1 = id * 1024 + (C & 31) * 32 + (R & 31);
+    }
+  }
   double acc[8] = {0, 0, 0, 0, 0, 0, 0, 0};
   int s = D.s0;
   for (; s + 8 <= D.s1; s += 8) {
@@ -38,10 +56,15 @@
   if (D.kind == 2) {
     double* base = lane < 6 ? gc : (lane < 12 ? wv : diagU);
     atomicAdd(&base[(size_t)D.dst * 6 + (lane % 6)], v);
+    if constexpr (kDirect) {
+      if (lane >= 12) atomicAdd(&T.diag_col[col], v);
+      else atomicAdd(&T.A[o0], lane < 6 ? -v : v);
+    }
+  } else if constexpr (kDirect) {
+    atomicAdd(&T.A[o0], v);
+    if (o1 >= 0) atomicAdd(&T.A[o1], v);
   } else {
     atomicAdd(&Sblk[(size_t)D.dst * 36 + lane], v);
-    if (D.kind == 1) {
-    }
   }
 }
 
@@ -49,8 +72,11 @@
   if (nchunks > 0) { count_launch(kLfTrackSweep); hipLaunchKernelGGL(k_track_sweep_dense, dim3(nchunks), dim3(kThreads), 0, s, a); }
 }
 void launch_reduce_slabs(const RedDest* dests, int ndest, const int32_t* srcs, const double* slab, double* Sblk, double* gc, double* wv, double* diagU,
-                         const LmCtl* ctl, hipStream_t s) {
-  if (ndest > 0) { count_launch(kLfReduceSlabs); hipLaunchKernelGGL(k_reduce_slabs, dim3((ndest + 3) / 4), dim3(256), 0, s, dests, ndest, srcs, slab, Sblk, gc, wv, diagU, ctl); }
+                         const LmCtl* ctl, hipStream_t s, const DirectAsm* direct) {
+  if (ndest <= 0) return;
+  count_launch(kLfReduceSlabs);
+  if (direct) hipLaunchKernelGGL(k_reduce_slabs<true>, dim3((ndest + 3) / 4), dim3(256), 0, s, dests, ndest, srcs, slab, Sblk, gc, wv, diagU, ctl, *direct);
+  else hipLaunchKernelGGL(k_reduce_slabs<false>, dim3((ndest + 3) / 4), dim3(256), 0, s, dests, ndest, srcs, slab, Sblk, gc, wv, diagU, ctl, DirectAsm{});
 }
 
 }
diff --git a/mpsfm_amd/csrc/sweep_dense_body.h b/mpsfm_amd/csrc/sweep_dense_body.h
--- a/mpsfm_amd/csrc/sweep_dense_body.h
+++ b/mpsfm_amd/csrc/sweep_dense_body.h
@@ -251,6 +251,11 @@
       adopt = A.ctl != nullptr && __builtin_amdgcn_readfirstlane(accepted) != 0;
       const int64_t g0 = (int64_t)(cix - A.chunk0) * kThreads + tid, gstep = (int64_t)A.nchunks * kThreads;
       for (int64_t e = g0; e < A.nred; e += gstep) A.red[e] = 0.0;
+#pragma unroll
+      for (int k = 0; k < 2; ++k)
+        for (int64_t e = g0; e < A.zero_n[k]; e += gstep) A.zero_p[k][e] = 0.0;
+      for (int64_t e = g0; e < (int64_t)A.zero_nptiles * 1024; e += gstep) A.zero_P[(int64_t)A.zero_ptiles[e >> 10] * 1024 + (e & 1023)] = 0.0;
+      for (int64_t e = gstep - 1 - g0; e < (int64_t)A.zero_ntiles * 1024; e += gstep) A.zero_A[(int64_t)A.zero_tiles[e >> 10] * 1024 + (e & 1023)] = 0.0;
       if (adopt) {
         for (int i = tid; i < 3 * npt; i += kThreads) A.pts_rw[(size_t)3 * H.pt0 + i] = A.pts2[(size_t)3 * H.pt0 + i];
         const int64_t n_q = 4 * (int64_t)A.adopt_nc, n_t = 3 * (int64_t)A.adopt_nc, n_tab = (int64_t)kCamRec * A.adopt_nc;
```
